# yaito3014/UECRayTracing

Measured on AMD Instinct MI355X. Metric: Msamples/sec at 1920x1080x512spp (~500 spheres); per-pixel RMSE vs CPU, higher is better.
Workload: dtype f64; 1 GPU; BASELINE config 3: 1920x1080x512spp, max_depth 50, RTIOW final scene (485 spheres, generator seed 42), seed0 404, mt19937 + FP64 bit-exact; image=1920x1080, spp=512, max_depth=50, spheres=485

## Files before the change

### uecraytracing_amd/csrc/yk_bvh.cpp

```cpp
#include "yk_bvh.hpp"

#include <algorithm>
#include <cmath>
#include <numeric>

namespace ykbvh {
namespace {

struct Box {
  double lo[3] = {INFINITY, INFINITY, INFINITY};
  double hi[3] = {-INFINITY, -INFINITY, -INFINITY};
  void grow(const Box& b) {
    for (int k = 0; k < 3; ++k) {
      lo[k] = std::min(lo[k], b.lo[k]);
      hi[k] = std::max(hi[k], b.hi[k]);
    }
  }
  void grow(const double* p) {
    for (int k = 0; k < 3; ++k) {
      lo[k] = std::min(lo[k], p[k]);
      hi[k] = std::max(hi[k], p[k]);
    }
  }
  double area() const {
    if (!(hi[0] >= lo[0])) return 0;
    const double dx = hi[0] - lo[0], dy = hi[1] - lo[1], dz = hi[2] - lo[2];
    return 2 * (dx * dy + dy * dz + dz * dx);
  }
};

struct Builder {
  const double* c;
  std::vector<Box> sbox;
  std::vector<double> cent;
  std::vector<uint32_t> idx;
  std::vector<Node> nodes;
  bool median_only = false;
  uint32_t max_depth = 0;
  Options opt;

  Box bounds(uint32_t b, uint32_t e) const {
    Box r;
    for (uint32_t i = b; i < e; ++i) r.grow(sbox[idx[i]]);
    return r;
  }

  int32_t rec(uint32_t b, uint32_t e, uint32_t depth) {
    const uint32_t n = e - b;
    if (n <= opt.max_leaf) {
      max_depth = std::max(max_depth, depth);
      return ~int32_t((b << 4) | n);
    }
    Box cb;
    for (uint32_t i = b; i < e; ++i) cb.grow(&cent[3 * idx[i]]);
    int axis = 0;
    for (int k = 1; k < 3; ++k)
      if (cb.hi[k] - cb.lo[k] > cb.hi[axis] - cb.lo[axis]) axis = k;
    uint32_t mid = b + n / 2;
    double ext = cb.hi[axis] - cb.lo[axis];
    if (!median_only && ext > 0) {
      const int kBins = std::min(std::max(opt.bins, 2), 256);
      double best = INFINITY;
      int best_q = -1, best_axis = axis;
      for (int ax = 0; ax < 3; ++ax) {
        if (!opt.all_axes && ax != axis) continue;
        const double ex = cb.hi[ax] - cb.lo[ax];
        if (!(ex > 0)) continue;
        std::vector<Box> bb(kBins);
        std::vector<uint32_t> cnt(kBins, 0);
        for (uint32_t i = b; i < e; ++i) {
          const uint32_t sp = idx[i];
          const int q = std::min(std::max(int((cent[3 * sp + ax] - cb.lo[ax]) / ex * kBins), 0), kBins - 1);
          bb[q].grow(sbox[sp]);
          ++cnt[q];
        }
        for (int q = 1; q < kBins; ++q) {
          Box l, r;
          uint32_t nl = 0, nr = 0;
          for (int t = 0; t < q; ++t) { l.grow(bb[t]); nl += cnt[t]; }
          for (int t = q; t < kBins; ++t) { r.grow(bb[t]); nr += cnt[t]; }
          if (!nl || !nr) continue;
          const double cost = l.area() * nl + r.area() * nr;
          if (cost < best) { best = cost; best_q = q; best_axis = ax; }
        }
      }
      axis = best_axis;
      ext = cb.hi[axis] - cb.lo[axis];
      auto bin_of = [&](uint32_t sp) {
        int q = int((cent[3 * sp + axis] - cb.lo[axis]) / ext * kBins);
        return std::min(std::max(q, 0), kBins - 1);
      };
      if (best_q > 0) {
        auto it = std::partition(idx.begin() + b, idx.begin() + e,
                                 [&](uint32_t sp) { return bin_of(sp) < best_q; });
        mid = uint32_t(it - idx.begin());
      }
    }
    if (mid == b || mid == e || median_only || ext == 0) {
      mid = b + n / 2;
      std::nth_element(idx.begin() + b, idx.begin() + mid, idx.begin() + e,
                       [&](uint32_t x, uint32_t y) { return cent[3 * x + axis] < cent[3 * y + axis]; });
    }
    const int32_t me = int32_t(nodes.size());
    nodes.emplace_back();
    const int32_t l = rec(b, mid, depth + 1);
    const int32_t r = rec(mid, e, depth + 1);
    const Box bl = bounds(b, mid), br = bounds(mid, e);
    Node& nd = nodes[me];
    const Box* kids[2] = {&bl, &br};
    for (int k = 0; k < 2; ++k) {
      auto dn = [](double v) { float f = (float)v; return (double)f > v ? std::nextafter(f, -INFINITY) : f; };
      auto up = [](double v) { float f = (float)v; return (double)f < v ? std::nextafter(f, INFINITY) : f; };
      nd.lo_x[k] = dn(kids[k]->lo[0]);
      nd.lo_y[k] = dn(kids[k]->lo[1]);
      nd.lo_z[k] = dn(kids[k]->lo[2]);
      nd.hi_x[k] = up(kids[k]->hi[0]);
      nd.hi_y[k] = up(kids[k]->hi[1]);
      nd.hi_z[k] = up(kids[k]->hi[2]);
    }
    nd.child[0] = l;
    nd.child[1] = r;
    nd.pad[0] = nd.pad[1] = 0;
    return me;
  }
};

}

Built build(const double* centers, const double* radii, uint32_t n, double camera_extent,
            const Options& opt) {
  Built out;
  double ext = camera_extent;
  for (uint32_t i = 0; i < n; ++i)
    for (int k = 0; k < 3; ++k) ext = std::max(ext, std::fabs(centers[3 * i + k]) + std::fabs(radii[i]));
  out.origin_bound = 4.0 * ext;
  out.delta = (float)std::ldexp(out.origin_bound, -21);
  for (int attempt = 0; attempt < 2; ++attempt) {
    Builder bd;
    bd.c = centers;
    bd.median_only = attempt == 1;
    bd.opt = opt;
    bd.sbox.resize(n);
    bd.cent.assign(centers, centers + 3 * size_t(n));
    bd.idx.resize(n);
    std::iota(bd.idx.begin(), bd.idx.end(), 0u);
    for (uint32_t i = 0; i < n; ++i) {
      const double ar = std::fabs(radii[i]);
      double g = ar * opt.radius_grow;
      if (opt.f32_big) {
        const double* c = centers + 3 * i;
        const double reach = std::sqrt(3.0) * out.origin_bound + std::sqrt(c[0] * c[0] + c[1] * c[1] + c[2] * c[2]) + ar;
        if (kF32BigReach * ar >= reach * (1.0 + 0x1p-20)) g = std::min(g, ar * kF32BigGrow);
      }
      const double r = ar + g + out.delta;
      for (int k = 0; k < 3; ++k) {
        bd.sbox[i].lo[k] = centers[3 * i + k] - r;
        bd.sbox[i].hi[k] = centers[3 * i + k] + r;
      }
    }
    out.root = bd.rec(0, n, 0);
    out.depth = bd.max_depth;
    if (out.depth <= kMaxDepth || attempt == 1) {
      out.nodes = std::move(bd.nodes);
      out.order = std::move(bd.idx);
      break;
    }
  }
  return out;
}


namespace {
struct Slot {
  float lo[3], hi[3];
  int32_t code;
};

float slot_area(const Slot& e) {
  const float dx = e.hi[0] - e.lo[0], dy = e.hi[1] - e.lo[1], dz = e.hi[2] - e.lo[2];
  return dx * dy + dy * dz + dz * dx;
}

Slot child_slot(const Node& n, int k) {
  return Slot{{n.lo_x[k], n.lo_y[k], n.lo_z[k]}, {n.hi_x[k], n.hi_y[k], n.hi_z[k]}, n.child[k]};
}

double box_area(const float* lo, const float* hi) {
  const double dx = (double)hi[0] - lo[0], dy = (double)hi[1] - lo[1], dz = (double)hi[2] - lo[2];
  return dx * dy + dy * dz + dz * dx;
}

double box_dist2(const float* lo, const float* hi, const double* p) {
  double d2 = 0;
  for (int a = 0; a < 3; ++a) {
    const double d = p[a] < lo[a] ? lo[a] - p[a] : (p[a] > hi[a] ? p[a] - hi[a] : 0.0);
    d2 += d * d;
  }
  return d2;
}

bool box_spans(const float* lo, const float* hi, const float* node_lo, const float* node_hi) {
  return box_area(lo, hi) >= kSpanArea * box_area(node_lo, node_hi);
}

struct Collapser {
  const Built& b;
  const WideOptions& opt;
  std::vector<WideNode>& out;
  std::vector<uint32_t> leaves;
  uint32_t max_depth = 0;

  uint32_t count_leaves(int32_t code) {
    if (code < 0) return 1;
    if (leaves.empty()) leaves.assign(b.nodes.size(), 0);
    if (leaves[code]) return leaves[code];
    return leaves[code] = count_leaves(b.nodes[code].child[0]) + count_leaves(b.nodes[code].child[1]);
  }
  double score(const Slot& e) {
    const double a = slot_area(e);
    if (opt.expand == 0) return a;
    const double nl = count_leaves(e.code);
    return opt.expand == 1 ? a * nl : a * std::sqrt(nl);
  }

  void order_slots(std::vector<Slot>& slots) const {
    if (!opt.view || opt.order == SlotOrder::kTree) return;
    float nlo[3] = {3e38f, 3e38f, 3e38f}, nhi[3] = {-3e38f, -3e38f, -3e38f};
    for (const Slot& e : slots)
      for (int a = 0; a < 3; ++a) {
        nlo[a] = std::min(nlo[a], e.lo[a]);
        nhi[a] = std::max(nhi[a], e.hi[a]);
      }
    struct Key {
      int low;
      double d2;
      Slot slot;
    };
    auto before = [](const Key& x, const Key& y) { return x.low != y.low ? x.low > y.low : x.d2 > y.d2; };
    Key keys[4];
    size_t n = 0;
    for (const Slot& e : slots) {
      const bool leaf = e.code < 0;
      const bool low = opt.order == SlotOrder::kNearLeavesLow
                           ? leaf
                           : (opt.order == SlotOrder::kNearSpanLow && leaf && box_spans(e.lo, e.hi, nlo, nhi));
      const Key key{low ? 1 : 0, box_dist2(e.lo, e.hi, opt.view), e};
      size_t at = n++;
      for (; at > 0 && before(key, keys[at - 1]); --at) keys[at] = keys[at - 1];
      keys[at] = key;
    }
    for (size_t k = 0; k < n; ++k) slots[k] = keys[k].slot;
  }

  uint32_t collapse(int32_t idx, uint32_t depth) {
    std::vector<Slot> slots = {child_slot(b.nodes[idx], 0), child_slot(b.nodes[idx], 1)};
    while (slots.size() < 4) {
      int best = -1;
      for (size_t i = 0; i < slots.size(); ++i)
        if (slots[i].code >= 0 && (best < 0 || score(slots[i]) > score(slots[best]))) best = (int)i;
      if (best < 0) break;
      const Node& c = b.nodes[slots[best].code];
      slots[best] = child_slot(c, 0);
      slots.insert(slots.begin() + best + 1, child_slot(c, 1));
    }
    order_slots(slots);
    max_depth = std::max(max_depth, depth + 1);
    const uint32_t me = (uint32_t)out.size();
    out.emplace_back();
    int32_t codes[4];
    for (int k = 0; k < 4; ++k) {
      if (k >= (int)slots.size()) {
        codes[k] = kEmptyLeaf;
      } else if (slots[k].code >= 0) {
        codes[k] = (int32_t)(collapse(slots[k].code, depth + 1) * sizeof(WideNode));
      } else {
        codes[k] = slots[k].code;
      }
    }
    WideNode& w = out[me];
    float* ax[3] = {w.x, w.y, w.z};
    for (int k = 0; k < 4; ++k) {
      const bool used = k < (int)slots.size();
      for (int a = 0; a < 3; ++a) {
        const float lo = used ? slots[k].lo[a] : 3e38f, hi = used ? slots[k].hi[a] : -3e38f;
        ax[a][k] = lo;
        ax[a][4 + k] = hi;
        ax[a][8 + k] = lo;
      }
      w.child[k] = codes[k];
    }
    return me;
  }
};

void slot_box(const WideNode& w, int k, float* lo, float* hi) {
  const float* ax[3] = {w.x, w.y, w.z};
  for (int a = 0; a < 3; ++a) {
    lo[a] = ax[a][k];
    hi[a] = ax[a][4 + k];
  }
}
}

bool slot_spans(const WideNode& w, int k) {
  float nlo[3] = {3e38f, 3e38f, 3e38f}, nhi[3] = {-3e38f, -3e38f, -3e38f}, lo[3], hi[3];
  for (int j = 0; j < 4; ++j) {
    slot_box(w, j, lo, hi);
    if (!(lo[0] <= hi[0])) continue;
    for (int a = 0; a < 3; ++a) {
      nlo[a] = std::min(nlo[a], lo[a]);
      nhi[a] = std::max(nhi[a], hi[a]);
    }
  }
  slot_box(w, k, lo, hi);
  return lo[0] <= hi[0] && box_spans(lo, hi, nlo, nhi);
}

double slot_dist2(const WideNode& w, int k, const double* p) {
  float lo[3], hi[3];
  slot_box(w, k, lo, hi);
  return box_dist2(lo, hi, p);
}

std::vector<WideNode> wide_nodes(const Built& b, int32_t* root_code, uint32_t* wide_depth,
                                 const WideOptions& wopt) {
  std::vector<WideNode> out;
  uint32_t depth = 0;
  if (b.root >= 0) {
    Collapser c{b, wopt, out, {}, 0};
    c.collapse(b.root, 0);
    depth = c.max_depth;
    *root_code = 0;
  } else {
    *root_code = b.root;
  }
  *wide_depth = depth;
  return out;
}

}
```

### uecraytracing_amd/csrc/yk_context.hip

```cpp
#include <hip/hip_runtime.h>

#include <algorithm>
#include <chrono>
#include <cmath>
#include <cstdio>
#include <cstdlib>
#include <cstring>
#include <string>
#include <vector>

#include "../../include/ykgpu.h"
#include "yk_host_internal.hpp"
#include "yk_schedule.hpp"

using namespace ykhost;

namespace {

thread_local std::string g_last_error;

__global__ void yk_mat_prep(SphereMat* m, uint32_t n) {
  const uint32_t i = blockIdx.x * blockDim.x + threadIdx.x;
  if (i < n) {
    m[i].inv_r = ykd::rcp_refined(m[i].radius);
    m[i].inv_rf = ykf::rcp_refined((float)m[i].radius);
  }
}

}

namespace ykhost {

int fail(int code, const std::string& msg) {
  g_last_error = msg;
  return code;
}
std::string& last_error() { return g_last_error; }

uint64_t device_bytes(const ykgpu_context* ctx) {
  uint64_t b = ctx->t64.bytes + ctx->t32.bytes;
  if (ctx->d_geo) b += (uint64_t)ctx->nspheres * (sizeof(SphereGeo) + sizeof(SphereMat) + sizeof(float4));
  b += ctx->warm_cap + ctx->col_cap * sizeof(double) + ctx->acc_cap * sizeof(double);
  b += ctx->retry_cap * sizeof(uint4);
  b += (uint64_t)ctx->order_slots * sizeof(uint32_t) + (uint64_t)ctx->counter_cap * sizeof(uint32_t);
  b += kCounters * sizeof(unsigned long long);
  if (ctx->d_mt) b += 2ull * ctx->scratch_lanes * ykd::kMtN * sizeof(uint32_t);
  if (ctx->d_ids) b += 2ull * ctx->id_lanes * ctx->id_stride * sizeof(uint16_t);
  b += ctx->rgb_cap + ctx->sums_cap * sizeof(double);
  b += (uint64_t)ctx->cast_cap * (sizeof(yk_ray) + sizeof(yk_hit));
  if (ctx->d_cast_counters) b += (uint64_t)kCastStripes * kCastCounters * sizeof(unsigned long long);
  b += (uint64_t)ctx->rad_cap * (sizeof(yk_path_ray) + sizeof(yk_radiance));
  if (ctx->d_rad_x397) b += kRadChunk * sizeof(uint32_t) + sizeof(uint32_t);
  b += (uint64_t)ctx->rad_mt_lanes * ykd::kMtN * sizeof(uint32_t);
  b += (uint64_t)ctx->rad_lanes * ctx->rad_id_stride * sizeof(uint16_t);
  if (ctx->d_rad_counters) b += (uint64_t)kRadStripes * kRadCounters * sizeof(unsigned long long);
  return b;
}

int finish_stats(ykgpu_context* ctx) {
  if (!ctx->stats_pending) return YK_OK;
  YK_HIP(hipEventSynchronize(ctx->ev1));
  float ms = 0;
  YK_HIP(hipEventElapsedTime(&ms, ctx->ev0, ctx->ev1));
  unsigned long long c[kCounters];
  YK_HIP(hipMemcpy(c, ctx->d_stats, sizeof(c), hipMemcpyDeviceToHost));
  ctx->stats.node_visits = c[4];
  ctx->stats.linear_scans = c[5];
  ctx->stats.newton_calls = c[6];
  ctx->stats.newton_iters = c[7];
  for (int k = 0; k < 8; ++k) ctx->stats.phase_cycles[k] = c[8 + k];
  for (int k = 0; k < 3; ++k) ctx->stats.timeline[k] = c[16 + k];
  for (int k = 0; k < 4; ++k) ctx->stats.diag[k] = c[19 + k];
  for (int k = 0; k < 8; ++k) ctx->stats.work[k] = c[24 + k];
  ctx->stats.total_ms = ms;
  double tw = 0, tr = 0, tp = 0, busy = 0;
  for (uint32_t k = 0; k + 5 < ctx->lev_used; k += 6) {
    float a = 0, b = 0, c = 0;
    YK_HIP(hipEventSynchronize(ctx->lev[k + 5]));
    YK_HIP(hipEventElapsedTime(&a, ctx->lev[k], ctx->lev[k + 1]));
    YK_HIP(hipEventElapsedTime(&b, ctx->lev[k + 2], ctx->lev[k + 3]));
    YK_HIP(hipEventElapsedTime(&c, ctx->lev[k + 4], ctx->lev[k + 5]));
    tw += a, tr += b, tp += c;
    float ov = 0;
    if (k >= 6) YK_HIP(hipEventElapsedTime(&ov, ctx->lev[k + 2], ctx->lev[k - 6 + 3]));
    busy += b - std::min<double>(b, std::max<double>(0.0, ov));
  }
  ctx->stats.render_busy_ms = busy;
  const uint32_t nl = ctx->lev_used / 6;
  std::vector<unsigned long long> clk(4ull * nl);
  std::vector<double> mhz(nl, 0.0);
  if (nl) YK_HIP(hipMemcpy(clk.data(), ctx->d_clk, clk.size() * sizeof(unsigned long long), hipMemcpyDeviceToHost));
  double cyc = 0, real = 0;
  for (uint32_t k = 0; k < nl; ++k) {
    const double dc = (double)(clk[4 * k + 2] - clk[4 * k]), dr = (double)(clk[4 * k + 3] - clk[4 * k + 1]);
    if (dr > 0 && clk[4 * k + 3] > clk[4 * k + 1]) {
      mhz[k] = dc / dr * 100.0;
      cyc += dc;
      real += dr;
    }
  }
  ctx->stats.sclk_mhz = real > 0 ? cyc / real * 100.0 : 0.0;
  if (std::getenv("YKGPU_TIMELINE")) {
    for (uint32_t k = 0; k + 5 < ctx->lev_prev_used && k + 5 < ctx->lev_prev.size(); k += 6) {
      float t[6];
      bool ok = true;
      for (int q = 0; q < 6 && ok; ++q) ok = hipEventElapsedTime(&t[q], ctx->ev0, ctx->lev_prev[k + q]) == hipSuccess;
      if (!ok) {
        (void)hipGetLastError();
        break;
      }
      std::fprintf(stderr, "prev   %u: warm %8.3f %8.3f  render %8.3f %8.3f  reduce %8.3f %8.3f\n", k / 6, t[0],
                   t[1], t[2], t[3], t[4], t[5]);
    }
    for (uint32_t k = 0; k + 5 < ctx->lev_used; k += 6) {
      float t[6];
      for (int q = 0; q < 6; ++q) YK_HIP(hipEventElapsedTime(&t[q], ctx->ev0, ctx->lev[k + q]));
      std::fprintf(stderr, "launch %u: warm %8.3f %8.3f  render %8.3f %8.3f  reduce %8.3f %8.3f  sclk %7.1f MHz\n",
                   k / 6, t[0], t[1], t[2], t[3], t[4], t[5], mhz[k / 6]);
    }
    std::fprintf(stderr, "call %8.3f\n", ms);
  }
  ctx->stats.warmup_ms = tw;
  ctx->stats.kernel_ms = tr;
  ctx->stats.resolve_ms = tp;
  ctx->stats.segments = c[0];
  ctx->stats.sphere_tests = c[1];
  ctx->stats.sqrt_calls = c[2];
  ctx->stats.mt_fallbacks = c[3];
  ctx->stats.device_bytes = device_bytes(ctx);
  ctx->stats_pending = false;
  return YK_OK;
}

}

namespace {

int upload_tree(ykgpu_context* ctx, DevTree& t, const std::vector<double>& centers, const std::vector<double>& radii,
                double cam_ext, const ykbvh::Options& opt, uint32_t leaf_cap, const void* geo, size_t elem,
                size_t tgeo_elem, const RenderKernel (&kern)[2][2], bool exact_stack,
                const ykbvh::WideOptions& wopt) {
  const uint32_t count = (uint32_t)radii.size();
  if (opt.max_leaf > leaf_cap) return fail(YK_ERR_UNSUPPORTED, "BVH leaf size above the kernel's leaf capacity");
  const ykbvh::Built bvh = ykbvh::build(centers.data(), radii.data(), count, cam_ext, opt);
  if (bvh.depth > ykbvh::kMaxDepth) return fail(YK_ERR_INVALID, "BVH deeper than the traversal stack");
  std::vector<char> leaf_geo(count * elem);
  for (uint32_t i = 0; i < count; ++i)
    std::memcpy(leaf_geo.data() + i * elem, (const char*)geo + (size_t)bvh.order[i] * elem, elem);
  t.release();
  int32_t root_code = 0;
  uint32_t wdepth = 0;
  const std::vector<DevNode> snodes = ykbvh::wide_nodes(bvh, &root_code, &wdepth, wopt);
  auto leaf_fits = [&](int32_t code) { return code >= 0 || (((~(uint32_t)code) & 15u) <= leaf_cap); };
  bool fits = leaf_fits(root_code);
  for (const DevNode& w : snodes)
    for (int k = 0; k < 4; ++k) fits = fits && leaf_fits(w.child[k]);
  if (!fits) return fail(YK_ERR_UNSUPPORTED, "a BVH leaf holds more spheres than the kernel's leaf code tests");
  const size_t nn = std::max<size_t>(1, snodes.size());
  YK_HIP(hipMalloc(&t.nodes, nn * sizeof(DevNode)));
  YK_HIP(hipMalloc(&t.leaf_geo, count * elem));
  YK_HIP(hipMalloc(&t.leaf_ids, count * sizeof(uint32_t)));
  if (!snodes.empty())
    YK_HIP(hipMemcpy(t.nodes, snodes.data(), snodes.size() * sizeof(DevNode), hipMemcpyHostToDevice));
  YK_HIP(hipMemcpy(t.leaf_geo, leaf_geo.data(), count * elem, hipMemcpyHostToDevice));
  YK_HIP(hipMemcpy(t.leaf_ids, bvh.order.data(), count * sizeof(uint32_t), hipMemcpyHostToDevice));
  t.bytes = nn * sizeof(DevNode) + count * elem + count * sizeof(uint32_t);
  t.root = root_code;
  t.depth = bvh.depth;
  t.wide_depth = wdepth;
  t.origin_bound = bvh.origin_bound;
  t.n_nodes = (uint32_t)snodes.size();
  auto a16 = [](size_t b) { return (b + 15) & ~size_t(15); };
  const size_t scene_bytes = a16(t.n_nodes * sizeof(DevNode)) + a16(count * elem) + a16(count * sizeof(uint32_t));
  const size_t tgeo_bytes = tgeo_elem ? a16(count * tgeo_elem) : 0;
  const size_t mat_bytes = tgeo_elem ? a16(count * sizeof(SphereMat)) : 0;
  t.geo_off = (uint32_t)a16(t.n_nodes * sizeof(DevNode));
  t.ids_off = t.geo_off + (uint32_t)a16(count * elem);
  for (int v = 0; v < 2; ++v) {
    DevTree::Plan& pl = t.plan[v];
    const int blk = block_of(v == 1);
    const int rays = blk;
    const size_t budget = (size_t)160 * 1024 / (blk >= 512 ? 1 : 768 / blk) - 2048;
    const size_t min_stacks = (size_t)12 * rays * 4;
    pl.in_lds = scene_bytes + tgeo_bytes + mat_bytes + min_stacks <= budget;
    const size_t tables = pl.in_lds ? tgeo_bytes + mat_bytes : 0;
    {
      const size_t used = pl.in_lds ? scene_bytes + tables : 0;
      const uint32_t fit = used + min_stacks <= budget ? (uint32_t)((budget - used) / (rays * 4)) : 12u;
      pl.stack_cap = std::max(8u, std::min(3 * wdepth + 1, fit - 4));
      pl.stack_entries = pl.stack_cap + 4;
      pl.stack_check = true;
      if (exact_stack && fit >= 3 * wdepth + 1) {
        pl.stack_cap = 3 * wdepth + 1;
        pl.stack_entries = pl.stack_cap;
        pl.stack_check = false;
      }
#ifdef YK_STACK_CAP_FORCE
      pl.stack_cap = YK_STACK_CAP_FORCE;
      pl.stack_entries = pl.stack_cap + 4;
      pl.stack_check = true;
#endif
    }
    pl.tgeo_off = pl.in_lds && tgeo_elem ? (uint32_t)scene_bytes : 0u;
    pl.mat_off = pl.in_lds && tgeo_elem ? (uint32_t)(scene_bytes + tgeo_bytes) : 0u;
    pl.stack_off = pl.in_lds ? (uint32_t)(scene_bytes + tables) : 0u;
    pl.lds_bytes = pl.stack_off + pl.stack_entries * rays * (uint32_t)sizeof(int32_t);
    int per_cu = 0;
    const RenderKernel k = kern[v][pl.in_lds ? 1 : 0];
    const hipError_t e = hipOccupancyMaxActiveBlocksPerMultiprocessor(&per_cu, k, blk, pl.lds_bytes);
    if (e != hipSuccess || per_cu < 1) per_cu = 1;
    pl.grid = per_cu * ctx->cus;
  }
  return YK_OK;
}

}

extern "C" {

uint32_t ykgpu_abi_version(void) { return YKGPU_ABI_VERSION; }

const char* ykgpu_last_error(void) { return g_last_error.c_str(); }

int ykgpu_device_count(int* count) {
  if (!count) return fail(YK_ERR_INVALID, "null count");
  int n = 0;
  hipError_t e = hipGetDeviceCount(&n);
  if (e != hipSuccess) {
    *count = 0;
    return fail(YK_ERR_DEVICE, std::string("hipGetDeviceCount: ") + hipGetErrorString(e));
  }
  *count = n;
  return YK_OK;
}

int ykgpu_context_create(int device, ykgpu_context** out) {
  if (!out) return fail(YK_ERR_INVALID, "null out");
  *out = nullptr;
  int n = 0;
  if (hipGetDeviceCount(&n) != hipSuccess || n == 0)
    return fail(YK_ERR_DEVICE, "no HIP device (the renderer has no CPU fallback)");
  if (device < 0 || device >= n) return fail(YK_ERR_INVALID, "device index out of range");
  YK_HIP(hipSetDevice(device));
  hipDeviceProp_t prop;
  YK_HIP(hipGetDeviceProperties(&prop, device));
  if (std::strncmp(prop.gcnArchName, "gfx950", 6) != 0)
    return fail(YK_ERR_DEVICE, std::string("built for gfx950, device is ") + prop.gcnArchName);
  auto* ctx = new ykgpu_context();
  ctx->device = device;
  ctx->cus = prop.multiProcessorCount;
  for (int k16 = 0; k16 < 16; ++k16)
    (void)hipFuncSetAttribute((const void*)fp64_kernel(k16 & 8, k16 & 7), hipFuncAttributeMaxDynamicSharedMemorySize,
                              160 * 1024);
  for (int k8 = 0; k8 < 8; ++k8)
    (void)hipFuncSetAttribute((const void*)f32_kernel(k8 & 4, (k8 & 1) | ((k8 & 2) << 1)),
                              hipFuncAttributeMaxDynamicSharedMemorySize, 160 * 1024);
  if (hipStreamCreateWithFlags(&ctx->stream, hipStreamNonBlocking) != hipSuccess ||
      hipStreamCreateWithFlags(&ctx->aux, hipStreamNonBlocking) != hipSuccess ||
      hipStreamCreateWithFlags(&ctx->red, hipStreamNonBlocking) != hipSuccess ||
      create_render_stream(&ctx->alt) != hipSuccess || create_render_stream(&ctx->ren) != hipSuccess ||
      hipEventCreate(&ctx->ev0) != hipSuccess || hipEventCreate(&ctx->ev1) != hipSuccess ||
      hipMalloc(&ctx->d_stats, kCounters * sizeof(unsigned long long)) != hipSuccess) {
    ykgpu_context_destroy(ctx);
    return fail(YK_ERR_DEVICE, "context resources");
  }
  *out = ctx;
  return YK_OK;
}

int ykgpu_context_destroy(ykgpu_context* ctx) {
  if (!ctx) return YK_OK;
  (void)hipSetDevice(ctx->device);
  if (ctx->stream) (void)hipStreamSynchronize(ctx->stream);
  (void)hipFree(ctx->d_geo);
  (void)hipFree(ctx->d_mat);
  (void)hipFree(ctx->d_geo_f);
  (void)hipFree(ctx->d_counter);
  (void)hipFree(ctx->d_clk);
  (void)hipFree(ctx->d_stats);
  (void)hipFree(ctx->d_warm);
  (void)hipFree(ctx->d_retry);
  (void)hipFree(ctx->d_order);
  (void)hipFree(ctx->d_col);
  (void)hipFree(ctx->d_acc);
  ctx->t64.release();
  ctx->t32.release();
  (void)hipFree(ctx->d_mt);
  (void)hipFree(ctx->d_ids);
  (void)hipFree(ctx->d_rgb);
  (void)hipFree(ctx->d_sums);
  (void)hipFree(ctx->d_cast_rays);
  (void)hipFree(ctx->d_cast_hits);
  (void)hipFree(ctx->d_cast_counters);
  if (ctx->cast_ev) (void)hipEventDestroy(ctx->cast_ev);
  for (void* q : {ctx->d_rad_rays, ctx->d_rad_out, (void*)ctx->d_rad_x397, (void*)ctx->d_rad_claim, (void*)ctx->d_rad_mt,
                  (void*)ctx->d_rad_ids, (void*)ctx->d_rad_counters})
    (void)hipFree(q);
  if (ctx->rad_ev) (void)hipEventDestroy(ctx->rad_ev);
  for (hipEvent_t e : ctx->lev) (void)hipEventDestroy(e);
  for (hipEvent_t e : ctx->lev_prev) (void)hipEventDestroy(e);
  for (hipEvent_t e : ctx->gev) (void)hipEventDestroy(e);
  if (ctx->ev0) (void)hipEventDestroy(ctx->ev0);
  if (ctx->ev1) (void)hipEventDestroy(ctx->ev1);
  if (ctx->stream) (void)hipStreamDestroy(ctx->stream);
  if (ctx->aux) (void)hipStreamDestroy(ctx->aux);
  if (ctx->red) (void)hipStreamDestroy(ctx->red);
  if (ctx->alt) (void)hipStreamDestroy(ctx->alt);
  if (ctx->ren) (void)hipStreamDestroy(ctx->ren);
  delete ctx;
  return YK_OK;
}

int ykgpu_set_scene(ykgpu_context* ctx, const yk_sphere* spheres, uint32_t count,
                    const yk_camera* camera) {
  if (!ctx || !spheres || !camera) return fail(YK_ERR_INVALID, "null argument");
  if (count == 0 || count > 65535) return fail(YK_ERR_INVALID, "sphere count must be 1..65535");
  std::vector<SphereGeo> geo(count);
  std::vector<SphereMat> mat(count);
  std::vector<float4> geo_f(count);
  for (uint32_t i = 0; i < count; ++i) {
    const yk_sphere& s = spheres[i];
    if (s.material > YK_MATERIAL_DIELECTRIC) return fail(YK_ERR_INVALID, "unknown material kind");
    geo[i] = {s.center[0], s.center[1], s.center[2], s.radius * s.radius};
    const float rf = (float)s.radius;
    geo_f[i] = make_float4((float)s.center[0], (float)s.center[1], (float)s.center[2], rf * rf);
    mat[i] = {s.albedo[0], s.albedo[1], s.albedo[2], s.fuzz, s.radius, s.ior, s.material, 0.0f, 0.0};
    if (s.material == YK_MATERIAL_DIELECTRIC) {
      const double inv = 1.0 / s.ior;
      double r0f = (1 - inv) / (1 + inv), r0b = (1 - s.ior) / (1 + s.ior);
      r0f = r0f * r0f;
      r0b = r0b * r0b;
      mat[i].fuzz = inv;
      mat[i].ar = r0f;
      mat[i].ag = r0b;
    }
  }
  YK_HIP(hipSetDevice(ctx->device));
  YK_HIP(hipEventSynchronize(ctx->ev1));
  YK_HIP(hipStreamSynchronize(ctx->stream));
  for (hipStream_t s : {ctx->aux, ctx->red, ctx->ren, ctx->alt}) YK_HIP(hipStreamSynchronize(s));
  if (ctx->cast_ev) YK_HIP(hipEventSynchronize(ctx->cast_ev));
  if (ctx->rad_ev) YK_HIP(hipEventSynchronize(ctx->rad_ev));
  ++ctx->scene_gen;
  if (count > ctx->nspheres || !ctx->d_geo) {
    (void)hipFree(ctx->d_geo);
    (void)hipFree(ctx->d_mat);
    (void)hipFree(ctx->d_geo_f);
    ctx->d_geo = nullptr;
    ctx->d_mat = nullptr;
    ctx->d_geo_f = nullptr;
    YK_HIP(hipMalloc(&ctx->d_geo, count * sizeof(SphereGeo)));
    YK_HIP(hipMalloc(&ctx->d_mat, count * sizeof(SphereMat)));
    YK_HIP(hipMalloc(&ctx->d_geo_f, count * sizeof(float4)));
  }
  YK_HIP(hipMemcpy(ctx->d_geo, geo.data(), count * sizeof(SphereGeo), hipMemcpyHostToDevice));
  YK_HIP(hipMemcpy(ctx->d_geo_f, geo_f.data(), count * sizeof(float4), hipMemcpyHostToDevice));
  std::vector<double> centers(3 * size_t(count)), radii(count);
  double rmin = INFINITY;
  for (uint32_t i = 0; i < count; ++i) {
    for (int k = 0; k < 3; ++k) centers[3 * i + k] = spheres[i].center[k];
    radii[i] = spheres[i].radius;
    rmin = std::min(rmin, std::fabs(radii[i]));
  }
  double cam_ext = 0;
  for (int k = 0; k < 3; ++k) cam_ext = std::max(cam_ext, std::fabs(camera->origin[k]));
  ykbvh::Options bopt;
  bopt.max_leaf = kLeafCapF64;
  if (const char* e = ab_knob("YKGPU_BVH_BINS")) bopt.bins = std::max(2, std::min(256, std::atoi(e)));
  bopt.all_axes = true;
  if (const char* e = ab_knob("YKGPU_BVH_ALLAXES")) bopt.all_axes = std::atoi(e) != 0;
  const RenderKernel k64[2][2] = {{fp64_kernel(false, 0), fp64_kernel(true, 0)},
                                  {fp64_kernel(false, 4), fp64_kernel(true, 4)}};
  ykbvh::WideOptions wopt;
  wopt.view = camera->origin;
  if (const char* e = ab_knob("YKGPU_BVH_ORDER"))
    wopt.order = (ykbvh::SlotOrder)std::max(0, std::min(3, std::atoi(e)));
  int rc = upload_tree(ctx, ctx->t64, centers, radii, cam_ext, bopt, kLeafCapF64, geo.data(), sizeof(SphereGeo),
                       sizeof(SphereGeo), k64, true, wopt);
  if (rc) return rc;
  {
    double dmax = 1.0;
    for (int k = 0; k < 3; ++k)
      dmax = std::max(dmax, std::fabs(camera->lower_left_corner[k]) + std::fabs(camera->horizontal[k]) +
                                std::fabs(camera->vertical[k]) + std::fabs(camera->origin[k]) +
                                std::fabs(camera->lens_radius) *
                                    (std::fabs(camera->lens_u[k]) + std::fabs(camera->lens_v[k])));
    if (!(ctx->t64.origin_bound <= 0x1p27) || !(ctx->t64.origin_bound >= 0x1p-60 * dmax))
      ctx->t64.origin_bound = -1.0;
  }
  ykbvh::Options fopt = bopt;
  fopt.max_leaf = kLeafCapF32;
  if (const char* e = ab_knob("YKGPU_BVH_ALLAXES_F32")) fopt.all_axes = std::atoi(e) != 0;
  fopt.radius_grow = 2.0 * (double)ykbvh::kF32Cone;
  fopt.f32_big = ab_knob("YKGPU_F32_NO_BIG") == nullptr;
  const RenderKernel k32[2][2] = {{f32_kernel(false, 0), f32_kernel(true, 0)},
                                  {f32_kernel(false, 4), f32_kernel(true, 4)}};
  ykbvh::WideOptions fwopt = wopt;
  if (const char* e = ab_knob("YKGPU_BVH_ORDER_F32"))
    fwopt.order = (ykbvh::SlotOrder)std::max(0, std::min(3, std::atoi(e)));
  rc = upload_tree(ctx, ctx->t32, centers, radii, cam_ext, fopt, kLeafCapF32, geo_f.data(), sizeof(float4),
                   sizeof(float4), k32, false, fwopt);
  if (rc) return rc;
  if (!(rmin >= 0x1p-20) || !(ctx->t32.origin_bound <= 0x1p20)) ctx->t32.origin_bound = -1.0;
  YK_HIP(hipMemcpy(ctx->d_mat, mat.data(), count * sizeof(SphereMat), hipMemcpyHostToDevice));
  hipLaunchKernelGGL(yk_mat_prep, dim3((count + 255) / 256), dim3(256), 0, ctx->stream, ctx->d_mat, count);
  YK_HIP(hipGetLastError());
  YK_HIP(hipStreamSynchronize(ctx->stream));
  ctx->nspheres = count;
  ctx->cam = *camera;
  double ext = 0;
  for (uint32_t i = 0; i < count; ++i) {
    const yk_sphere& s = spheres[i];
    const double e = std::fmax(std::fabs(s.center[0]), std::fmax(std::fabs(s.center[1]), std::fabs(s.center[2]))) +
                     std::fabs(s.radius);
    ext = e > ext || e != e ? e : ext;
    if (ext != ext) break;
  }
  ctx->cast_extent = ext;
  ctx->have_scene = true;
  return YK_OK;
}

int ykgpu_render_async(ykgpu_context* ctx, const yk_render_params* p, void* rgb_device,
                       void* stream) {
  int rc = check_params(ctx, p);
  if (rc) return rc;
  if (!rgb_device) return fail(YK_ERR_INVALID, "null output");
  YK_HIP(hipSetDevice(ctx->device));
  hipStream_t st = stream ? (hipStream_t)stream : ctx->stream;
  ctx->t0 = std::chrono::steady_clock::now();
  return launch(ctx, p, (uint8_t*)rgb_device, nullptr, st, 0, p->samples_per_pixel, nullptr);
}

static int render_host(ykgpu_context* ctx, const yk_render_params* p, uint8_t* rgb_host,
                       double* sums_host) {
  int rc = check_params(ctx, p);
  if (rc) return rc;
  YK_HIP(hipSetDevice(ctx->device));
  const auto t0 = std::chrono::steady_clock::now();
  const size_t npix = (size_t)p->row_count * tile_width(p);
  if (npix * 3 > ctx->rgb_cap) {
    (void)hipFree(ctx->d_rgb);
    ctx->d_rgb = nullptr;
    YK_HIP(hipMalloc(&ctx->d_rgb, npix * 3));
    ctx->rgb_cap = npix * 3;
  }
  if (sums_host && npix * 3 > ctx->sums_cap) {
    (void)hipFree(ctx->d_sums);
    ctx->d_sums = nullptr;
    YK_HIP(hipMalloc(&ctx->d_sums, npix * 3 * sizeof(double)));
    ctx->sums_cap = npix * 3;
  }
  rc = launch(ctx, p, ctx->d_rgb, sums_host ? ctx->d_sums : nullptr, ctx->stream, 0, p->samples_per_pixel, nullptr);
  if (rc) return rc;
  if (rgb_host) YK_HIP(hipMemcpyAsync(rgb_host, ctx->d_rgb, npix * 3, hipMemcpyDeviceToHost, ctx->stream));
  if (sums_host)
    YK_HIP(hipMemcpyAsync(sums_host, ctx->d_sums, npix * 3 * sizeof(double), hipMemcpyDeviceToHost,
                          ctx->stream));
  YK_HIP(hipStreamSynchronize(ctx->stream));
  rc = finish_stats(ctx);
  ctx->stats.total_ms =
      std::chrono::duration<double, std::milli>(std::chrono::steady_clock::now() - t0).count();
  return rc;
}

int ykgpu_render(ykgpu_context* ctx, const yk_render_params* p, uint8_t* rgb_host) {
  if (!rgb_host) return fail(YK_ERR_INVALID, "null output");
  return render_host(ctx, p, rgb_host, nullptr);
}

int ykgpu_render_trace(ykgpu_context* ctx, const yk_render_params* p, uint32_t max_rays, double* rays_host,
                       uint32_t* counts_host) {
  int rc = check_params(ctx, p);
  if (rc) return rc;
  if (!max_rays || !rays_host || !counts_host) return fail(YK_ERR_INVALID, "null output or max_rays == 0");
  const size_t n = (size_t)p->row_count * tile_width(p) * p->samples_per_pixel;
  YK_HIP(hipSetDevice(ctx->device));
  YK_HIP(hipMalloc(&ctx->d_trace, n * max_rays * 6 * sizeof(double)));
  if (hipMalloc(&ctx->d_trace_counts, n * sizeof(uint32_t)) != hipSuccess) {
    (void)hipFree(ctx->d_trace);
    ctx->d_trace = nullptr;
    return fail(YK_ERR_NOMEM, "ykgpu_render_trace: ray counts");
  }
  ctx->trace_cap = max_rays;
  yk_render_params q = *p;
  q.flags |= YK_FLAG_COUNT_WORK | YK_FLAG_TRACE_RAYS;
  rc = render_host(ctx, &q, nullptr, nullptr);
  hipError_t e = hipSuccess;
  if (!rc) e = hipMemcpy(rays_host, ctx->d_trace, n * max_rays * 6 * sizeof(double), hipMemcpyDeviceToHost);
  if (!rc && e == hipSuccess) e = hipMemcpy(counts_host, ctx->d_trace_counts, n * sizeof(uint32_t), hipMemcpyDeviceToHost);
  (void)hipFree(ctx->d_trace);
  (void)hipFree(ctx->d_trace_counts);
  ctx->d_trace = nullptr;
  ctx->d_trace_counts = nullptr;
  ctx->trace_cap = 0;
  if (rc) return rc;
  if (e != hipSuccess) return fail(YK_ERR_DEVICE, std::string("ykgpu_render_trace: ") + hipGetErrorString(e));
  return YK_OK;
}

int ykgpu_render_sums(ykgpu_context* ctx, const yk_render_params* p, double* sums_host) {
  if (!sums_host) return fail(YK_ERR_INVALID, "null output");
  return render_host(ctx, p, nullptr, sums_host);
}

int ykgpu_get_stats(ykgpu_context* ctx, yk_render_stats* out) {
  if (!ctx || !out) return fail(YK_ERR_INVALID, "null argument");
  YK_HIP(hipSetDevice(ctx->device));
  int rc = finish_stats(ctx);
  if (rc) return rc;
  *out = ctx->stats;
  return YK_OK;
}

}
```

### uecraytracing_amd/csrc/yk_device.hpp

```cpp
#pragma once

#include <hip/hip_runtime.h>
#include <stdint.h>

namespace ykd {

struct v3 {
  double x, y, z;
};
__device__ __forceinline__ v3 add(v3 a, v3 b) { return {a.x + b.x, a.y + b.y, a.z + b.z}; }
__device__ __forceinline__ v3 sub(v3 a, v3 b) { return {a.x - b.x, a.y - b.y, a.z - b.z}; }
__device__ __forceinline__ v3 mul(v3 a, double s) { return {a.x * s, a.y * s, a.z * s}; }
__device__ __forceinline__ v3 divs(v3 a, double s) { return {a.x / s, a.y / s, a.z / s}; }
__device__ __forceinline__ v3 neg(v3 a) { return {-a.x, -a.y, -a.z}; }
__device__ __forceinline__ double dot(v3 a, v3 b) { return a.x * b.x + a.y * b.y + a.z * b.z; }
__device__ __forceinline__ double len2(v3 a) { return a.x * a.x + a.y * a.y + a.z * a.z; }

__device__ __forceinline__ bool div_range(double x) { return fabs(x) >= 0x1p-400 && fabs(x) <= 0x1p400; }
__device__ __forceinline__ bool num_range(double x) { return x == 0.0 || div_range(x); }
__device__ __forceinline__ double rcp_refined(double s) {
  const double r0 = __builtin_amdgcn_rcp(s);
  double t = __builtin_fma(-s, r0, 1.0);
  const double r1 = __builtin_fma(r0, t, r0);
  t = __builtin_fma(-s, r1, 1.0);
  return __builtin_fma(r1, t, r1);
}
__device__ __forceinline__ double div_by(double n, double s, double r) {
  const double q0 = n * r;
  const double e = __builtin_fma(-s, q0, n);
  return __builtin_copysign(__builtin_fma(e, r, q0), q0);
}
__device__ __forceinline__ double div_pos(double n, double s, double r) {
  const double q0 = n * r;
  return __builtin_fma(__builtin_fma(-s, q0, n), r, q0);
}
__device__ __forceinline__ v3 divs_fast(v3 a, double s) {
  const double r = rcp_refined(s);
  v3 q = {div_by(a.x, s, r), div_by(a.y, s, r), div_by(a.z, s, r)};
  const bool ok = div_range(s) && num_range(a.x) && num_range(a.y) && num_range(a.z);
  if (__builtin_expect(__ballot(!ok) != 0, 0)) q = divs(a, s);
  return q;
}
__device__ __forceinline__ v3 divs_fast_r(v3 a, double s, double r) {
  v3 q = {div_by(a.x, s, r), div_by(a.y, s, r), div_by(a.z, s, r)};
  const bool ok = div_range(s) && num_range(a.x) && num_range(a.y) && num_range(a.z);
  if (__builtin_expect(__ballot(!ok) != 0, 0)) q = divs(a, s);
  return q;
}
__device__ __forceinline__ double div_markstein(double n, double d, double y) {
  const double q0 = n * y;
  return __builtin_fma(__builtin_fma(-d, q0, n), y, q0);
}

__device__ __forceinline__ double sqrt_bound(double x) {
  const double r = __builtin_amdgcn_rsq(x);
  const double y = x * r, h = 0.5 * r;
  const double y1 = __builtin_fma(__builtin_fma(-y, y, x), h, y);
  return x == 0.0 ? 0.0 : y1;
}
__device__ __forceinline__ double rcp_bound(double a) {
  const double r0 = __builtin_amdgcn_rcp(a);
  return __builtin_fma(r0, __builtin_fma(-a, r0, 1.0), r0);
}
__device__ __forceinline__ double sqrt_start(double s) {
  const double r = __builtin_amdgcn_rsq(s);
  double g = s * r, h = r * 0.5;
  const double e = __builtin_fma(-h, g, 0.5);
  g = __builtin_fma(g, e, g);
  h = __builtin_fma(h, e, h);
  double d = __builtin_fma(-g, g, s);
  g = __builtin_fma(d, h, g);
  d = __builtin_fma(-g, g, s);
  return __builtin_fma(d, h, g);
}

__device__ __forceinline__ double nsqrt_impl(double s, uint32_t& iters) {
  double x, prev = 0.0;
  if (s >= 0x1p-400 && s <= 0x1p400) {
    x = sqrt_start(s);
    ++iters;
    return (x + div_pos(s, x, rcp_refined(x))) / 2.0;
  }
  x = (s >= 0x1p-1000 && s <= 0x1.fffffffffffffp+1023) ? __builtin_sqrt(s) : s / 2.0;
  for (int guard = 0; x != prev && guard < 4096; ++guard) {
    prev = x;
    x = (x + s / x) / 2.0;
    ++iters;
  }
  return x;
}
__device__ __forceinline__ double nsqrt(double s) {
  uint32_t it = 0;
  return nsqrt_impl(s, it);
}

__device__ __forceinline__ double nsqrt_c(double s, uint32_t& calls, uint32_t& iters) {
  ++calls;
  return nsqrt_impl(s, iters);
}

__device__ __forceinline__ v3 normalized(v3 a) { return divs(a, nsqrt(len2(a))); }
__device__ __forceinline__ v3 reflect(v3 v, v3 n) { return sub(v, mul(n, 2.0 * dot(v, n))); }
__device__ __forceinline__ bool near_zero(v3 a) {
  const double ax = a.x > 0 ? a.x : -a.x, ay = a.y > 0 ? a.y : -a.y;
  return (ax < 1e-8) && (ay < 1e-8) && (ax < 1e-8);
}

constexpr uint32_t kMtN = 624, kMtM = 397, kLazyDraws = kMtN - kMtM;

__device__ __forceinline__ uint32_t mt_seed_step(uint32_t prev, uint32_t i) {
  return 1812433253u * (prev ^ (prev >> 30)) + i;
}
__device__ __forceinline__ uint32_t xor_and(uint32_t a, uint32_t b, uint32_t c) {
  return __builtin_amdgcn_bitop3_b32(a, b, c, 0x78);
}
__device__ __forceinline__ uint32_t mt_mix(uint32_t hi_src, uint32_t lo_src) {
  const uint32_t y = __builtin_amdgcn_bitop3_b32(hi_src, lo_src, 0x80000000u, 0xE4);
  const uint32_t odd = 0u - (lo_src & 1u);
  return xor_and(y >> 1, odd, 0x9908b0dfu);
}
__device__ __forceinline__ uint32_t mt_temper(uint32_t z) {
  z ^= (z >> 11);
  z = xor_and(z, z << 7, 0x9d2c5680u);
  z = xor_and(z, z << 15, 0xefc60000u);
  z ^= (z >> 18);
  return z;
}

struct MtLane {
  uint32_t a0, a1, b;
  uint32_t j;
  uint32_t seed;
  uint32_t* state;
};
__device__ __forceinline__ bool mt_used_fallback(const MtLane& g) { return g.j > kLazyDraws; }
__device__ __forceinline__ uint32_t rng_words(const MtLane& g) { return g.j; }
__device__ __forceinline__ uint32_t rng_twists(const MtLane& g) { return g.j > kLazyDraws ? 1u + (g.j - 1u) / kMtN : 0u; }

__device__ __forceinline__ void mt_start(MtLane& g, uint32_t seed) {
  g.seed = seed;
  g.j = 0;
  g.a0 = seed;
  uint32_t x = mt_seed_step(seed, 1);
  g.a1 = x;
#pragma unroll 8
  for (uint32_t i = 2; i <= kMtM; ++i) x = mt_seed_step(x, i);
  g.b = x;
}

__device__ __forceinline__ void mt_start_from(MtLane& g, uint32_t seed, uint32_t x397) {
  g.seed = seed;
  g.j = 0;
  g.a0 = seed;
  g.a1 = mt_seed_step(seed, 1);
  g.b = x397;
}

#ifndef YK_WALK_MAD
#define YK_WALK_MAD 1
#endif
__device__ __forceinline__ uint32_t mt_seed_step_mad(uint32_t prev, uint64_t i, uint32_t cmul) {
  const uint32_t t = prev ^ (prev >> 30);
  uint64_t r, carry;
  asm("v_mad_u64_u32 %0, %1, %2, %3, %4" : "=v"(r), "=s"(carry) : "v"(t), "v"(cmul), "s"(i));
  return (uint32_t)r;
}

template <int N>
__device__ __forceinline__ void mt_walk397xn(uint32_t (&x)[N]) {
#pragma unroll
  for (int k = 0; k < N; ++k) x[k] = mt_seed_step(x[k], 1);
#if YK_WALK_MAD
  uint32_t cmul;
  asm("v_mov_b32 %0, 0x6c078965" : "=v"(cmul));
#pragma unroll 4
  for (uint32_t i = 2; i <= kMtM; ++i) {
#pragma unroll
    for (int k = 0; k < N; ++k) x[k] = mt_seed_step_mad(x[k], (uint64_t)i, cmul);
  }
#else
#pragma unroll 4
  for (uint32_t i = 2; i <= kMtM; ++i) {
#pragma unroll
    for (int k = 0; k < N; ++k) x[k] = mt_seed_step(x[k], i);
  }
#endif
}

constexpr uint32_t kMtSeedMulInv = 0x9638806du;
__device__ __forceinline__ uint32_t mt_seed_from(uint32_t x, uint32_t i) {
  for (; i > 0; --i) {
    const uint32_t t = (x - i) * kMtSeedMulInv;
    x = t ^ (t >> 30);
  }
  return x;
}
__device__ __noinline__ uint32_t mt_slow(uint32_t* st, uint32_t x227, uint32_t j) {
  const uint32_t idx = j % kMtN;
  if (j == kLazyDraws) {
    uint32_t x = mt_seed_from(x227, kLazyDraws);
    st[0] = x;
    for (uint32_t i = 1; i < kMtN; ++i) {
      x = mt_seed_step(x, i);
      st[i] = x;
    }
  }
  if (j == kLazyDraws || idx == 0) {
    uint32_t k = 0;
    for (; k < kMtN - kMtM; ++k) st[k] = st[k + kMtM] ^ mt_mix(st[k], st[k + 1]);
    for (; k < kMtN - 1; ++k) st[k] = st[k + kMtM - kMtN] ^ mt_mix(st[k], st[k + 1]);
    st[kMtN - 1] = st[kMtM - 1] ^ mt_mix(st[kMtN - 1], st[0]);
  }
  return st[idx];
}

__device__ __forceinline__ uint32_t mt_next_lazy(MtLane& g) {
  const uint32_t z = g.b ^ mt_mix(g.a0, g.a1);
  g.a0 = g.a1;
  g.a1 = mt_seed_step(g.a1, g.j + 2);
  g.b = mt_seed_step(g.b, g.j + kMtM + 1);
  ++g.j;
  return mt_temper(z);
}
__device__ __forceinline__ bool rng_lazy_ok(const MtLane& g, uint32_t words) { return g.j + words <= kLazyDraws; }

__device__ __forceinline__ uint32_t mt_next(MtLane& g) {
  uint32_t z;
  if (g.j < kLazyDraws) {
    z = g.b ^ mt_mix(g.a0, g.a1);
    g.a0 = g.a1;
    g.a1 = mt_seed_step(g.a1, g.j + 2);
    g.b = mt_seed_step(g.b, g.j + kMtM + 1);
  } else {
    z = mt_slow(g.state, g.a0, g.j);
  }
  ++g.j;
  return mt_temper(z);
}

__device__ __forceinline__ uint32_t sample_seed(uint32_t mode, uint64_t key, uint32_t seed0, uint32_t y,
                                                uint32_t x, uint32_t W, uint32_t spp, uint32_t s) {
#ifndef YK_SEED_COUNTER_ONLY
  if (mode == 1u) {
    uint64_t z = key + (((uint64_t)y * W + x) * spp + s + 1) * 0x9E3779B97F4A7C15ull;
    z = (z ^ (z >> 30)) * 0xBF58476D1CE4E5B9ull;
    z = (z ^ (z >> 27)) * 0x94D049BB133111EBull;
    z ^= z >> 31;
    return (uint32_t)(z >> 32);
  }
#endif
  return seed0 + (y * W + x) * spp + s;
}

struct X128Lane {
  uint32_t x, y, z, w;
  uint32_t n;
};
__device__ __forceinline__ void x128_start(X128Lane& g, uint32_t seed) {
  g.x = 123456789u;
  g.y = 362436069u;
  g.z = 521288629u;
  g.w = 88675123u ^ seed;
  g.n = 0;
}
__device__ __forceinline__ uint32_t x128_next(X128Lane& g) {
  const uint32_t t = g.x ^ (g.x << 11);
  g.x = g.y;
  g.y = g.z;
  g.z = g.w;
  g.w = (g.w ^ (g.w >> 19)) ^ (t ^ (t >> 8));
  ++g.n;
  return g.w;
}
__device__ __forceinline__ bool mt_used_fallback(const X128Lane&) { return false; }
__device__ __forceinline__ uint32_t rng_words(const X128Lane& g) { return g.n; }
__device__ __forceinline__ uint32_t rng_twists(const X128Lane&) { return 0u; }

__device__ __forceinline__ bool rng_lazy_ok(const X128Lane&, uint32_t) { return true; }

template <bool kLazy = false>
__device__ __forceinline__ uint32_t rng_next(MtLane& g) { return kLazy ? mt_next_lazy(g) : mt_next(g); }
template <bool kLazy = false>
__device__ __forceinline__ uint32_t rng_next(X128Lane& g) { return x128_next(g); }

template <bool kLazy = false, class G>
__device__ __forceinline__ double canonical(G& g) {
  const double u0 = (double)rng_next<kLazy>(g);
  const double u1 = (double)rng_next<kLazy>(g);
  double r = __builtin_fma(u1, 0x1p-32, u0 * 0x1p-64);
  if (r >= 1.0) r = 1.0 - 0x1p-53;
  return r;
}
template <bool kLazy = false, class G>
__device__ __forceinline__ double uniform(G& g, double a, double b) {
  return (canonical<kLazy>(g) * (b - a)) + a;
}
__device__ __forceinline__ double uniform_of(double c, double a, double b) {
  if (a == -1.0 && b == 1.0) return __builtin_fma(c, 2.0, -1.0);
  if (a == 0.0 && b == 1.0) return c;
  return (c * (b - a)) + a;
}
__device__ __forceinline__ bool rng_can_speculate(const MtLane& g) { return g.j + 2 <= kLazyDraws; }
__device__ __forceinline__ bool rng_can_speculate(const X128Lane&) { return true; }
template <class G>
__device__ __forceinline__ v3 random_vec(G& g, double lo, double hi) {
  v3 r;
  r.x = uniform(g, lo, hi);
  r.y = uniform(g, lo, hi);
  r.z = uniform(g, lo, hi);
  return r;
}

__device__ __forceinline__ double reflectance_r0(double cosine, double r0) {
  const double x = 1 - cosine;
  return r0 + (1 - r0) * ((((x * x) * x) * x) * x);
}

}
```

### uecraytracing_amd/csrc/yk_host_internal.hpp

```cpp
#ifndef YK_HOST_INTERNAL_HPP
#define YK_HOST_INTERNAL_HPP

#include <hip/hip_runtime.h>

#include <chrono>
#include <cstdint>
#include <map>
#include <string>
#include <vector>

#include "../../include/ykgpu.h"
#include "yk_render_device.hpp"

namespace ykhost {
int fail(int code, const std::string& msg);
std::string& last_error();
}

#define YK_HIP(call)                                                                      \
  do {                                                                                    \
    hipError_t e_ = (call);                                                               \
    if (e_ != hipSuccess)                                                                 \
      return ykhost::fail(e_ == hipErrorOutOfMemory ? YK_ERR_NOMEM : YK_ERR_DEVICE,       \
                          std::string(#call) + ": " + hipGetErrorString(e_));             \
  } while (0)

struct DevTree {
  DevNode* nodes = nullptr;
  void* leaf_geo = nullptr;
  uint32_t* leaf_ids = nullptr;
  int32_t root = 0;
  uint32_t depth = 0, n_nodes = 0;
  uint32_t wide_depth = 0;
  double origin_bound = 0;
  uint32_t geo_off = 0, ids_off = 0;
  size_t bytes = 0;
  struct Plan {
    bool in_lds = false;
    uint32_t lds_bytes = 0, stack_off = 0, stack_cap = 0, stack_entries = 0;
    bool stack_check = true;
    uint32_t tgeo_off = 0, mat_off = 0;
    int grid = 0;
  } plan[2];
  void release() {
    (void)hipFree(nodes);
    (void)hipFree(leaf_geo);
    (void)hipFree(leaf_ids);
    nodes = nullptr;
    leaf_geo = nullptr;
    leaf_ids = nullptr;
    bytes = 0;
  }
};

constexpr int kCastCounters = 8, kCastStripes = 64;
constexpr int kRadCounters = 8, kRadStripes = 64;
constexpr uint64_t kRadChunk = 1ull << 22;

struct ykgpu_context {
  int device = 0;
  int cus = 0;
  DevTree t64, t32;
  size_t scratch_lanes = 0;
  char* d_warm = nullptr;
  uint4* d_retry = nullptr;
  size_t retry_cap = 0;
  double* d_col = nullptr;
  double* d_acc = nullptr;
  size_t col_cap = 0, acc_cap = 0;
  uint32_t* d_order = nullptr;
  uint32_t order_w = 0, order_rows = 0, order_slots = 0, order_stride = 0, order_mode = 0;
  size_t warm_cap = 0;
  hipStream_t stream = nullptr;
  hipStream_t aux = nullptr;
  hipStream_t red = nullptr;
  hipStream_t alt = nullptr;
  hipStream_t ren = nullptr;
  hipEvent_t ev0 = nullptr, ev1 = nullptr;
  std::vector<hipEvent_t> lev;
  uint32_t lev_used = 0;
  std::vector<hipEvent_t> lev_prev;
  uint32_t lev_prev_used = 0;
  uint32_t prev_n = 0;
  std::vector<hipEvent_t> gev;
  uint64_t run_len = 0;
  struct RingGeom {
    uint64_t nps = 0, K = 0, welem = 0, warm_ring = 0, col_ring = 0, lanes = 0, id_stride = 0;
    const void *warm = nullptr, *col = nullptr, *mt = nullptr, *ids = nullptr;
    bool operator==(const RingGeom& o) const {
      return nps == o.nps && K == o.K && welem == o.welem && warm_ring == o.warm_ring && col_ring == o.col_ring &&
             lanes == o.lanes && id_stride == o.id_stride && warm == o.warm && col == o.col && mt == o.mt &&
             ids == o.ids;
    }
  } prev_geom;
  uint64_t prev_shape = 0;
  bool prev_ok = false;
  bool prev_enqueued = false;
  bool dirty = false;
  uint64_t g_next = 0;
  SphereGeo* d_geo = nullptr;
  SphereMat* d_mat = nullptr;
  float4* d_geo_f = nullptr;
  uint32_t nspheres = 0;
  yk_camera cam{};
  bool have_scene = false;
  uint64_t scene_gen = 0;
  uint32_t* d_counter = nullptr;
  uint32_t counter_cap = 0;
  unsigned long long* d_clk = nullptr;
  unsigned long long* d_stats = nullptr;
  uint32_t* d_mt = nullptr;
  uint16_t* d_ids = nullptr;
  uint32_t id_stride = 0;
  size_t id_lanes = 0;
  uint8_t* d_rgb = nullptr;
  size_t rgb_cap = 0;
  double* d_sums = nullptr;
  size_t sums_cap = 0;
  yk_render_stats stats{};
  bool stats_pending = false;
  double* d_trace = nullptr;
  uint32_t* d_trace_counts = nullptr;
  uint32_t trace_cap = 0;
  std::chrono::steady_clock::time_point t0;
  double cast_extent = 0;
  void* d_cast_rays = nullptr;
  void* d_cast_hits = nullptr;
  size_t cast_cap = 0;
  unsigned long long* d_cast_counters = nullptr;
  hipEvent_t cast_ev = nullptr;
  yk_cast_stats cast_stats{};
  void* d_rad_rays = nullptr;
  void* d_rad_out = nullptr;
  size_t rad_cap = 0;
  uint32_t* d_rad_x397 = nullptr;
  uint32_t* d_rad_claim = nullptr;
  uint32_t* d_rad_mt = nullptr;
  uint16_t* d_rad_ids = nullptr;
  size_t rad_lanes = 0, rad_id_stride = 0, rad_mt_lanes = 0;
  unsigned long long* d_rad_counters = nullptr;
  hipEvent_t rad_ev = nullptr;
  yk_radiance_stats rad_stats{};
};

struct ykgpu_film {
  ykgpu_context* ctx = nullptr;
  int device = 0;
  yk_render_params p{};
  uint64_t scene_gen = 0;
  uint32_t done = 0;
  uint32_t nps = 0;
  uint64_t npix = 0;
  double* d_plane = nullptr;
  uint32_t* d_order = nullptr;
  unsigned long long* d_result = nullptr;
  std::vector<uint32_t> order;
  bool torn = false;
  std::map<uint32_t, uint64_t> hist;
  uint32_t* d_count = nullptr;
  uint32_t* d_take = nullptr;
  uint32_t* d_blocks = nullptr;
  uint32_t* d_gorder = nullptr;
  uint32_t* d_gmap = nullptr;
  unsigned long long* d_hist = nullptr;
  uint32_t g_slots = 0;
  void* d_denoise = nullptr;
  void* d_features = nullptr;
  uint32_t feature_grid = 0;
  bool uniform() const { return hist.size() <= 1; }
};

struct ykgpu_group {
  std::vector<ykgpu_context*> ctx;
  std::vector<uint8_t*> tile;
  std::vector<size_t> tile_cap;
  std::vector<yk_render_stats> st;
  yk_render_stats total{};
};

struct ykgpu_group_film {
  ykgpu_group* g = nullptr;
  yk_render_params p{};
  uint32_t k = 0, wt = 0;
  std::vector<ykgpu_film*> film;
  std::vector<uint32_t> rows;
  std::vector<uint64_t> gen;
  std::vector<ykgpu_film*> band;
  uint32_t halo = 0;
  bool have_bands = false;
  bool torn = false;
};

namespace {
inline RenderKernel fp64_kernel(bool lds, int mode) { return (RenderKernel)yk_fp64_kernel(lds, mode); }
inline RenderKernel f32_kernel(bool lds, int mode) { return (RenderKernel)yk_f32_kernel(lds, mode); }
}

namespace ykhost {

int check_params(const ykgpu_context* ctx, const yk_render_params* p);
uint32_t tile_width(const yk_render_params* p);
uint64_t host_row_y(const yk_render_params* p, uint32_t t);
uint64_t host_col_x(const yk_render_params* p, uint32_t j);
uint32_t order_mode();
uint32_t order_stride(const yk_render_params* p);
std::vector<uint32_t> build_order(uint32_t W, uint32_t rows, uint32_t stride, uint32_t mode);
hipError_t create_render_stream(hipStream_t* s);
int launch(ykgpu_context* ctx, const yk_render_params* p, uint8_t* rgb_dev, double* sums_dev, hipStream_t st,
           uint32_t s_begin, uint32_t s_end, ykgpu_film* film);
uint64_t device_bytes(const ykgpu_context* ctx);
int finish_stats(ykgpu_context* ctx);
int film_ready(const ykgpu_film* film);
int film_accumulate_enqueue(ykgpu_film* film, uint32_t n_samples);
int film_accumulate_finish(ykgpu_film* film, uint32_t n_samples, std::chrono::steady_clock::time_point t0);
int denoise_params_check(const yk_denoise_params& dp);
int feature_params_check(const yk_feature_params& fp);
struct DenoiseBufs {
  double *mv, *out;
  uint8_t* rgb;
  unsigned long long* low;
};
int denoise_buffers(ykgpu_film* film, DenoiseBufs* out);
hipError_t denoise_moments_enqueue(ykgpu_film* film, const DenoiseBufs& b);
hipError_t denoise_band_enqueue(ykgpu_film* band, const DenoiseBufs& b, const yk_denoise_params& dp,
                                const yk_feature_params* fp, const double* feat, uint32_t r0, uint32_t n, bool want_rgb);
int yk_film_features_ensure(ykgpu_film* film, uint32_t grid, const double** planes, double* ms);

inline const uint32_t* film_counts(const ykgpu_film* film) { return film->uniform() ? nullptr : film->d_count; }
inline bool film_consecutive(const ykgpu_film* film) {
  const yk_render_params& p = film->p;
  return host_row_y(&p, p.row_count - 1) == (uint64_t)p.row_begin + p.row_count - 1 &&
         host_col_x(&p, tile_width(&p) - 1) == (uint64_t)p.col_begin + tile_width(&p) - 1;
}
struct TileCols {
  uint32_t begin, stride, band;
};
inline TileCols film_cols(const ykgpu_film* film) {
  const yk_render_params& p = film->p;
  return p.col_count ? TileCols{p.col_begin, p.col_stride, p.col_band_log2} : TileCols{0, 1, 0};
}

}

#endif
```

### uecraytracing_amd/csrc/yk_pipeline.hip

```cpp
#include <hip/hip_runtime.h>

#include <algorithm>
#include <cmath>
#include <cstdlib>
#include <random>
#include <string>
#include <vector>

#include "../../include/ykgpu.h"
#include "yk_film_internal.hpp"
#include "yk_host_internal.hpp"
#include "yk_schedule.hpp"

namespace {

struct WarmArgs {
  uint32_t W, spp, seed0, row_begin, row_stride, s0, npix_slots, seed_mode, band_log2;
  uint32_t Wt, col_begin, col_stride, col_band;
  uint32_t nps_m, nps_sh, w_m, w_sh;
  uint32_t lens, H;
  uint64_t seed_key;
  yk_camera cam;
  CamF camf;
  double w_d, h_d, inv_w, inv_h;
  const uint32_t* order;
  uint64_t n;
  void* out;
  uint32_t* counter;
  uint4* retry;
  uint32_t retry_cap, retry_pad;
};

inline uint32_t retry_cap_for(uint64_t slots_per_wave) {
  const double m = 0.2146 * (double)slots_per_wave, sd = std::sqrt(m * 0.7854);
  return ((uint32_t)(m + 6.0 * sd) + 64u + 63u) & ~63u;
}
__device__ __forceinline__ void retry_put(uint4* r, uint32_t i, const ykd::MtLane& g, double uc, double vc) {
  r[0] = make_uint4(i, g.seed, g.a0, g.a1);
  r[1] = make_uint4(g.b, g.j, 0u, 0u);
  *(double2*)(r + 2) = make_double2(uc, vc);
}
__device__ __forceinline__ uint64_t ld_l2(const uint4* r, int k) {
  return __hip_atomic_load((const uint64_t*)r + k, __ATOMIC_RELAXED, __HIP_MEMORY_SCOPE_AGENT);
}
__device__ __forceinline__ uint32_t retry_get(const uint4* r, ykd::MtLane& g, double& uc, double& vc) {
  const uint64_t w0 = ld_l2(r, 0), w1 = ld_l2(r, 1), w2 = ld_l2(r, 2);
  g.state = nullptr;
  g.seed = (uint32_t)(w0 >> 32);
  g.a0 = (uint32_t)w1;
  g.a1 = (uint32_t)(w1 >> 32);
  g.b = (uint32_t)w2;
  g.j = (uint32_t)(w2 >> 32);
  uc = __longlong_as_double((long long)ld_l2(r, 4));
  vc = __longlong_as_double((long long)ld_l2(r, 5));
  return (uint32_t)w0;
}

template <bool kLens, bool kF32, bool kDefer, uint32_t kIlp>
__device__ __forceinline__ void mt_warmup_body(const WarmArgs& wa) {
  constexpr uint32_t kWarmBlock = 256;
  const uint32_t n = (uint32_t)wa.n;
  const uint32_t stride = gridDim.x * kWarmBlock;
  if (blockIdx.x == 0 && threadIdx.x == 0) *wa.counter = 0u;
  static_assert(!kDefer || (kLens && !kF32), "the deferred lens loop is the FP64 lens warm-up's");
  uint4* const ring =
      kDefer ? wa.retry + (size_t)__builtin_amdgcn_readfirstlane((blockIdx.x * kWarmBlock + threadIdx.x) >> 6) *
                              wa.retry_cap * 3
             : nullptr;
  uint32_t rcount = 0;
  auto slot_seed = [&](uint32_t i, uint32_t& xx, uint32_t& y) -> uint32_t {
    const uint32_t sl = fdiv(i, wa.nps_m, wa.nps_sh), pp = i - sl * wa.npix_slots;
    const uint32_t q = wa.order[pp];
    const uint32_t pix = q == kNoPixel ? 0u : q;
    const uint32_t tr = fdiv(pix, wa.w_m, wa.w_sh);
    xx = tile_col_x(wa.col_begin, wa.col_stride, wa.col_band, pix - tr * wa.Wt);
    y = tile_row_y(wa.row_begin, wa.row_stride, wa.band_log2, tr);
    const uint32_t seed = ykd::sample_seed(wa.seed_mode, wa.seed_key, wa.seed0, y, xx, wa.W, wa.spp, wa.s0 + sl);
    xx = q == kNoPixel ? kPadX : xx;
    return seed;
  };
  auto start_slot = [&](uint32_t i, uint32_t xx, uint32_t y, uint32_t seed, uint32_t x397) {
    ykd::MtLane g;
    g.state = nullptr;
    ykd::mt_start_from(g, seed, x397);
    bool failed = false;
    if constexpr (kF32) {
      const float uc = ykf::canonical<true>(g);
      const float vc = ykf::canonical<true>(g);
      float px = 0.0f, py = 0.0f;
      if (kLens) {
        for (;;) {
          if (!ykd::rng_lazy_ok(g, 2)) {
            failed = true;
            break;
          }
          px = ykf::uniform_of(ykf::canonical<true>(g), -1.0f, 1.0f);
          py = ykf::uniform_of(ykf::canonical<true>(g), -1.0f, 1.0f);
          if (px * px + py * py < 1.0f) break;
        }
      }
      ykf::v3 o, d;
      camera_ray_f32(wa.camf, wa.H, xx, y, uc, vc, kLens, px, py, o, d);
      uint4* const out = (uint4*)wa.out + 3 * (size_t)i;
      *(float4*)out = make_float4(o.x, o.y, o.z, d.x);
      *(float4*)(out + 1) = make_float4(d.y, d.z, 0.0f, 0.0f);
      out[2] = make_uint4(g.a0, g.a1, g.b, xx == kPadX ? kPadSlot : failed ? kNoStart : g.j);
    } else {
      const double uc = ykd::canonical<true>(g);
      const double vc = ykd::canonical<true>(g);
      double px = 0.0, py = 0.0;
      if constexpr (kDefer) {
        bool again = false;
        if (!ykd::rng_lazy_ok(g, 4)) {
          failed = true;
        } else {
          px = ykd::uniform<true>(g, -1, 1);
          py = ykd::uniform<true>(g, -1, 1);
          again = !(px * px + py * py < 1.0);
        }
        const unsigned long long m = __ballot(again);
        const uint32_t nq = (uint32_t)__popcll(m);
        const bool room = rcount + nq <= wa.retry_cap;
        if (room) {
          if (again) {
            const uint32_t pos = rcount + __builtin_amdgcn_mbcnt_hi((uint32_t)(m >> 32), __builtin_amdgcn_mbcnt_lo((uint32_t)m, 0u));
            retry_put(ring + 3 * pos, i, g, uc, vc);
          }
          rcount += nq;
          if (again) return;
        } else if (again) {
          failed = true;
        }
      } else if (kLens) {
        for (;;) {
          if (!ykd::rng_lazy_ok(g, 4)) {
            failed = true;
            break;
          }
          px = ykd::uniform<true>(g, -1, 1);
          py = ykd::uniform<true>(g, -1, 1);
          if (px * px + py * py < 1.0) break;
        }
      }
      v3 o, d;
      camera_ray(wa.cam, wa.w_d, wa.inv_w, wa.h_d, wa.inv_h, wa.H, xx, y, uc, vc, kLens, px, py, o, d);
      uint4* const out = (uint4*)wa.out + 4 * (size_t)i;
      *(double2*)out = make_double2(o.x, o.y);
      *(double2*)(out + 1) = make_double2(o.z, d.x);
      *(double2*)(out + 2) = make_double2(d.y, d.z);
      out[3] = make_uint4(g.a0, g.a1, g.b, xx == kPadX ? kPadSlot : failed ? kNoStart : g.j);
    }
  };
  if constexpr (kIlp > 1) {
    for (uint32_t i = blockIdx.x * kWarmBlock + threadIdx.x; i < n; i += kIlp * stride) {
      uint32_t xx, y, x[kIlp];
#pragma unroll
      for (uint32_t k = kIlp - 1; k > 0; --k) {
        const uint32_t ik = i + k * stride;
        x[k] = slot_seed(ik < n ? ik : i, xx, y);
      }
      const uint32_t seed = slot_seed(i, xx, y);
      x[0] = seed;
      ykd::mt_walk397xn<kIlp>(x);
      start_slot(i, xx, y, seed, x[0]);
#pragma unroll
      for (uint32_t k = 1; k < kIlp; ++k) {
        const uint32_t ik = i + k * stride;
        if (ik < n) {
          const uint32_t sk = slot_seed(ik, xx, y);
          start_slot(ik, xx, y, sk, x[k]);
        }
      }
    }
  } else {
    for (uint32_t i = blockIdx.x * kWarmBlock + threadIdx.x; i < n; i += stride) {
      uint32_t xx, y;
      const uint32_t seed = slot_seed(i, xx, y);
      uint32_t x[1] = {seed};
      ykd::mt_walk397xn<1>(x);
      start_slot(i, xx, y, seed, x[0]);
    }
  }
  if constexpr (kDefer) {
    const uint32_t lane = threadIdx.x & 63u;
    uint32_t head = 0, cnt = __builtin_amdgcn_readfirstlane(rcount);
    asm volatile("s_waitcnt vmcnt(0)" ::: "memory");
    while (cnt > 0u) {
      const uint32_t take = min(cnt, 64u);
      const bool act = lane < take;
      ykd::MtLane g;
      double uc = 0, vc = 0, px = 0, py = 0;
      uint32_t i = 0;
      bool again = false, failed = false;
      if (act) {
        uint32_t pos = head + lane;
        pos = pos >= wa.retry_cap ? pos - wa.retry_cap : pos;
        i = retry_get(ring + 3 * pos, g, uc, vc);
        if (!ykd::rng_lazy_ok(g, 4)) {
          failed = true;
        } else {
          px = ykd::uniform<true>(g, -1, 1);
          py = ykd::uniform<true>(g, -1, 1);
          again = !(px * px + py * py < 1.0);
        }
      }
      head += take;
      head = head >= wa.retry_cap ? head - wa.retry_cap : head;
      cnt -= take;
      const unsigned long long m = __ballot(again);
      if (again) {
        uint32_t pos = head + cnt + __builtin_amdgcn_mbcnt_hi((uint32_t)(m >> 32), __builtin_amdgcn_mbcnt_lo((uint32_t)m, 0u));
        pos = pos >= wa.retry_cap ? pos - wa.retry_cap : pos;
        retry_put(ring + 3 * pos, i, g, uc, vc);
      }
      cnt += (uint32_t)__popcll(m);
      if (act && !again) {
        const uint32_t sl = fdiv(i, wa.nps_m, wa.nps_sh), pp = i - sl * wa.npix_slots;
        const uint32_t q = wa.order[pp];
        const uint32_t pix = q == kNoPixel ? 0u : q;
        const uint32_t tr = fdiv(pix, wa.w_m, wa.w_sh);
        const uint32_t xx = tile_col_x(wa.col_begin, wa.col_stride, wa.col_band, pix - tr * wa.Wt);
        const uint32_t y = tile_row_y(wa.row_begin, wa.row_stride, wa.band_log2, tr);
        uint4* const out = (uint4*)wa.out + 4 * (size_t)i;
        out[3] = make_uint4(g.a0, g.a1, g.b, q == kNoPixel ? kPadSlot : failed ? kNoStart : g.j);
        v3 o, d;
        camera_ray(wa.cam, wa.w_d, wa.inv_w, wa.h_d, wa.inv_h, wa.H, xx, y, uc, vc, kLens, px, py, o, d);
        *(double2*)out = make_double2(o.x, o.y);
        *(double2*)(out + 1) = make_double2(o.z, d.x);
        *(double2*)(out + 2) = make_double2(d.y, d.z);
      }
      if (cnt > 0u) asm volatile("s_waitcnt vmcnt(0)" ::: "memory");
    }
  }
}

template <bool kLens, bool kF32>
__global__ __launch_bounds__(256) void yk_mt_warmup(WarmArgs wa) {
  mt_warmup_body<kLens, kF32, false, 1>(wa);
}
__global__ __launch_bounds__(256) __attribute__((amdgpu_num_vgpr(YK_DEFER_VGPRS / 2))) void yk_mt_warmup_defer(WarmArgs wa) {
  mt_warmup_body<true, false, true, kWalkIlp>(wa);
}

struct ReduceArgs {
  const double* col;
  double* acc;
  const uint32_t* order;
  uint8_t* rgb;
  double* sums;
  uint32_t npix_slots, nsl, ks, spp;
  uint32_t first, last, pad0, pad1;
};
__device__ __forceinline__ void reduce_slot(const ReduceArgs& ra, uint32_t p) {
  const uint32_t q = ra.order[p];
  if (q == kNoPixel) return;
  double a[3];
#pragma unroll
  for (int c = 0; c < 3; ++c) a[c] = ra.first ? 0.0 : ra.acc[(size_t)c * ra.npix_slots + p];
  for (uint32_t k = 0; k < ra.ks; ++k) {
    const size_t i = (size_t)k * ra.npix_slots + p;
#pragma unroll
    for (int c = 0; c < 3; ++c) a[c] = a[c] + ra.col[i * kColStride + c];
  }
  if (!ra.last) {
#pragma unroll
    for (int c = 0; c < 3; ++c) ra.acc[(size_t)c * ra.npix_slots + p] = a[c];
    return;
  }
  const size_t o3 = (size_t)q * 3;
  const double spp = (double)ra.spp;
#pragma unroll
  for (int c = 0; c < 3; ++c) {
    if (ra.sums) ra.sums[o3 + c] = a[c];
    double v = ykd::nsqrt(a[c] / spp);
    v = (v < 0.0) ? 0.0 : (0.999 < v) ? 0.999 : v;
    ra.rgb[o3 + c] = (uint8_t)(uint32_t)(v * 256);
  }
}
__global__ __launch_bounds__(256) void yk_reduce_samples(ReduceArgs ra) {
  for (uint32_t p = blockIdx.x * blockDim.x + threadIdx.x; p < ra.npix_slots; p += gridDim.x * blockDim.x)
    reduce_slot(ra, p);
}

struct FilmReduceArgs {
  const double* col;
  double* plane;
  const uint32_t* order;
  uint32_t npix_slots, ks;
};
__global__ __launch_bounds__(256) void yk_film_reduce(FilmReduceArgs fa) {
  for (uint32_t p = blockIdx.x * blockDim.x + threadIdx.x; p < fa.npix_slots; p += gridDim.x * blockDim.x) {
    if (fa.order[p] == kNoPixel) continue;
    double s[3], q[3];
#pragma unroll
    for (int c = 0; c < 3; ++c) {
      s[c] = fa.plane[(size_t)c * fa.npix_slots + p];
      q[c] = fa.plane[(size_t)(3 + c) * fa.npix_slots + p];
    }
    for (uint32_t k = 0; k < fa.ks; ++k) {
      const double* rec = fa.col + ((size_t)k * fa.npix_slots + p) * kColStride;
#pragma unroll
      for (int c = 0; c < 3; ++c) {
        const double v = rec[c];
        s[c] = film_add(s[c], v);
        q[c] = film_add(q[c], film_mul(v, v));
      }
    }
#pragma unroll
    for (int c = 0; c < 3; ++c) {
      fa.plane[(size_t)c * fa.npix_slots + p] = s[c];
      fa.plane[(size_t)(3 + c) * fa.npix_slots + p] = q[c];
    }
  }
}

struct FilmMaskedArgs {
  const double* col;
  double* plane;
  uint32_t* count;
  uint32_t* take;
  const uint32_t* map;
  uint32_t npix_slots, g_slots, ks, pad;
};
__global__ __launch_bounds__(256) void yk_film_reduce_masked(FilmMaskedArgs fa) {
  for (uint32_t a = blockIdx.x * blockDim.x + threadIdx.x; a < fa.g_slots; a += gridDim.x * blockDim.x) {
    const uint32_t p = fa.map[a];
    if (p >= fa.npix_slots) continue;
    double s[3], q[3];
#pragma unroll
    for (int c = 0; c < 3; ++c) {
      s[c] = fa.plane[(size_t)c * fa.npix_slots + p];
      q[c] = fa.plane[(size_t)(3 + c) * fa.npix_slots + p];
    }
    for (uint32_t k = 0; k < fa.ks; ++k) {
      const double* rec = fa.col + ((size_t)k * fa.g_slots + a) * kColStride;
#pragma unroll
      for (int c = 0; c < 3; ++c) {
        const double v = rec[c];
        s[c] = film_add(s[c], v);
        q[c] = film_add(q[c], film_mul(v, v));
      }
    }
#pragma unroll
    for (int c = 0; c < 3; ++c) {
      fa.plane[(size_t)c * fa.npix_slots + p] = s[c];
      fa.plane[(size_t)(3 + c) * fa.npix_slots + p] = q[c];
    }
    fa.count[p] += fa.ks;
    if (fa.take) fa.take[p] = 0u;
  }
}

}

static_assert(kLaunchBytes / (8 * kColStride) * 4 < (1ull << 32), "4 * slot must fit 32 bits");
static_assert(yksched::kColourBytes == kColStride * sizeof(double), "yk_schedule.hpp's colour record");

namespace ykhost {

uint64_t host_row_y(const yk_render_params* p, uint32_t t) {
  const uint32_t L = p->row_band_log2;
  return (uint64_t)p->row_begin + ((((uint64_t)(t >> L)) * p->row_stride) << L) + (t & ((1u << L) - 1u));
}

uint32_t tile_width(const yk_render_params* p) { return p->col_count ? p->col_count : p->image_width; }
uint64_t host_col_x(const yk_render_params* p, uint32_t j) {
  if (!p->col_count) return j;
  const uint32_t L = p->col_band_log2;
  return (uint64_t)p->col_begin + ((((uint64_t)(j >> L)) * p->col_stride) << L) + (j & ((1u << L) - 1u));
}

static void fastdiv(uint32_t d, uint32_t& m, uint32_t& sh) {
  uint32_t l = 0;
  while ((1ull << l) < d) ++l;
  sh = 31 + l;
  m = (uint32_t)(((1ull << sh) + d - 1) / d);
}

int check_params(const ykgpu_context* ctx, const yk_render_params* p) {
  if (!ctx || !p) return fail(YK_ERR_INVALID, "null context or params");
  if (!ctx->have_scene) return fail(YK_ERR_NO_SCENE, "ykgpu_set_scene was not called");
  if (!p->image_width || !p->image_height || !p->samples_per_pixel)
    return fail(YK_ERR_INVALID, "image_width, image_height and samples_per_pixel must be > 0");
  if (!p->row_count) return fail(YK_ERR_INVALID, "row_count must be > 0");
  if (!p->row_stride) return fail(YK_ERR_INVALID, "row_stride must be > 0");
  if (p->row_band_log2 > 10) return fail(YK_ERR_INVALID, "row_band_log2 must be <= 10");
  if (host_row_y(p, p->row_count - 1) >= p->image_height) return fail(YK_ERR_INVALID, "row range outside the image");
  if (p->col_count) {
    if (!p->col_stride) return fail(YK_ERR_INVALID, "col_stride must be > 0");
    if (p->col_band_log2 > 10) return fail(YK_ERR_INVALID, "col_band_log2 must be <= 10");
    if (host_col_x(p, p->col_count - 1) >= p->image_width) return fail(YK_ERR_INVALID, "column range outside the image");
  } else if (p->col_begin || p->col_stride || p->col_band_log2) {
    return fail(YK_ERR_INVALID, "col_count == 0 (every column) needs col_begin, col_stride, col_band_log2 == 0");
  }
  if ((uint64_t)p->row_count * tile_width(p) >= (1ull << 31))
    return fail(YK_ERR_INVALID, "tile larger than 2^31 pixels");
  if (p->precision != YK_PRECISION_FP64 && p->precision != YK_PRECISION_FP32)
    return fail(YK_ERR_UNSUPPORTED, "precision mode");
  if (p->rng != YK_RNG_MT19937 && p->rng != YK_RNG_XOR128) return fail(YK_ERR_UNSUPPORTED, "rng mode");
  if (p->seed_mode != YK_SEED_COUNTER && p->seed_mode != YK_SEED_RANDOM_DEVICE)
    return fail(YK_ERR_UNSUPPORTED, "seed mode");
  if (!(p->t_min >= 0)) return fail(YK_ERR_INVALID, "t_min must be >= 0");
  if ((p->flags & YK_FLAG_ONE_LANE) &&
      (!(p->flags & YK_FLAG_COUNT_WORK) || p->precision != YK_PRECISION_FP64))
    return fail(YK_ERR_INVALID, "YK_FLAG_ONE_LANE needs YK_FLAG_COUNT_WORK and FP64");
  return YK_OK;
}

static int quiesce(ykgpu_context* ctx) {
  for (hipStream_t s : {ctx->aux, ctx->red, ctx->ren, ctx->alt, ctx->stream}) YK_HIP(hipStreamSynchronize(s));
  return YK_OK;
}

static int ensure_scratch(ykgpu_context* ctx, uint32_t max_depth, size_t lanes, bool need_mt) {
  if (need_mt && (lanes > ctx->scratch_lanes || !ctx->d_mt)) {
    if (int rc = quiesce(ctx)) return rc;
    (void)hipFree(ctx->d_mt);
    ctx->d_mt = nullptr;
    ctx->scratch_lanes = 0;
    YK_HIP(hipMalloc(&ctx->d_mt, 2 * lanes * ykd::kMtN * sizeof(uint32_t)));
    ctx->scratch_lanes = lanes;
  }
  const uint32_t need = max_depth > kStackRegs ? max_depth : 1;
  if (need > ctx->id_stride || lanes > ctx->id_lanes || !ctx->d_ids) {
    if (int rc = quiesce(ctx)) return rc;
    if (ctx->d_ids) YK_HIP(hipFree(ctx->d_ids));
    ctx->d_ids = nullptr;
    ctx->id_stride = 0;
    ctx->id_lanes = 0;
    YK_HIP(hipMalloc(&ctx->d_ids, 2 * lanes * need * sizeof(uint16_t)));
    ctx->id_stride = need;
    ctx->id_lanes = lanes;
  }
  return YK_OK;
}

uint32_t order_mode() {
  const char* oe = ab_knob("YKGPU_ORDER");
  return oe ? (uint32_t)std::atoi(oe) : 0u;
}
uint32_t order_stride(const yk_render_params* p) {
  return p->row_count > 1 && p->row_band_log2 < 3 ? p->row_stride : 1;
}
std::vector<uint32_t> build_order(uint32_t W, uint32_t rows, uint32_t stride, uint32_t mode) {
  std::vector<uint32_t> ord;
  if (kTile == 0) {
    ord.resize((size_t)W * rows);
    for (size_t i = 0; i < ord.size(); ++i) ord[i] = (uint32_t)i;
  } else {
    const uint32_t th = stride <= 1 ? kTile : (stride <= 4 ? std::max(1u, kTile / 2) : std::max(1u, kTile / 4));
    const uint32_t tw = kTile * kTile / th;
    const uint32_t bx = (W + tw - 1) / tw, by = (rows + th - 1) / th;
    ord.reserve((size_t)bx * by * tw * th);
    for (uint32_t jj = 0; jj < by; ++jj)
      for (uint32_t i = 0; i < bx; ++i)
        for (uint32_t k = 0; k < tw * th; ++k) {
          const uint32_t j = mode == 1 ? by - 1 - jj : jj;
          const uint32_t x = i * tw + k % tw, y = j * th + k / tw;
          ord.push_back(x < W && y < rows ? y * W + x : kNoPixel);
        }
  }
  return ord;
}
static int ensure_order(ykgpu_context* ctx, uint32_t W, uint32_t rows, uint32_t stride) {
  const uint32_t mode = order_mode();
  if (ctx->d_order && ctx->order_w == W && ctx->order_rows == rows && ctx->order_stride == stride &&
      ctx->order_mode == mode)
    return YK_OK;
  const std::vector<uint32_t> ord = build_order(W, rows, stride, mode);
  if (int rc = quiesce(ctx)) return rc;
  (void)hipFree(ctx->d_order);
  ctx->d_order = nullptr;
  ctx->order_w = ctx->order_rows = ctx->order_slots = 0;
  YK_HIP(hipMalloc(&ctx->d_order, ord.size() * sizeof(uint32_t)));
  YK_HIP(hipMemcpy(ctx->d_order, ord.data(), ord.size() * sizeof(uint32_t), hipMemcpyHostToDevice));
  ctx->order_w = W;
  ctx->order_rows = rows;
  ctx->order_stride = stride;
  ctx->order_mode = mode;
  ctx->order_slots = (uint32_t)ord.size();
  return YK_OK;
}

hipError_t create_render_stream(hipStream_t* s) {
  int least = 0, greatest = 0;
  const char* e = ab_knob("YKGPU_RENDER_PRIO");
  if ((e && std::atoi(e) == 0) || hipDeviceGetStreamPriorityRange(&least, &greatest) != hipSuccess)
    return hipStreamCreateWithFlags(s, hipStreamNonBlocking);
  return hipStreamCreateWithPriority(s, hipStreamNonBlocking, greatest);
}

static uint32_t col_ring() {
  uint32_t r = YK_COL_RING;
  if (const char* e = ab_knob("YKGPU_COL_RING")) r = (uint32_t)std::max(2, std::min(8, std::atoi(e)));
  return r;
}

static uint32_t reduce_blocks(const ykgpu_context* ctx, uint32_t nps) {
  uint32_t cap = (uint32_t)ctx->cus * 4;
  if (const char* e = ab_knob("YKGPU_RED_BLOCKS")) cap = (uint32_t)std::max(0, std::atoi(e));
  const uint32_t full = (nps + 255) / 256;
  return cap ? std::max(1u, std::min(full, cap)) : full;
}

static uint32_t warm_per_cu(bool f32) {
  uint32_t per_cu = f32 ? 2u : (uint32_t)YK_WARM_PER_CU;
  if (const char* e = ab_knob("YKGPU_WARM_PER_CU")) per_cu = (uint32_t)std::max(1, std::atoi(e));
  return per_cu;
}
inline uint32_t warm_blocks_for(uint64_t n, uint64_t cap, uint32_t ilp) {
  uint64_t wb = std::min<uint64_t>((n + 256 * kWarmSlots - 1) / (256 * kWarmSlots), cap);
  if (ilp > 1 && wb > 0) {
    const uint64_t per = 256ull * ilp, it = (n + wb * per - 1) / (wb * per);
    wb = (n + per * it - 1) / (per * it);
  }
  return (uint32_t)wb;
}


struct LaunchPlan {
  bool f32, x128;
  bool group;
  const DevTree* tree;
  const DevTree::Plan* plan;
  int grid, block;
  uint64_t seed_key;
  const uint32_t* order;
  uint32_t nps;
  uint32_t spp;
  std::vector<std::pair<uint32_t, uint32_t>> sched;
  uint64_t shape;
  bool warm_first;
  uint32_t K, nlaunch, kWarmRing, kColRing, mem_shrinks;
  size_t welem;
  uint32_t retry_cap;
  size_t retry_n;
};

static uint64_t warm_wave_slots(const ykgpu_context* ctx, uint64_t nl) {
  const uint64_t wb = warm_blocks_for(nl, (uint64_t)ctx->cus * warm_per_cu(false), kWalkIlp);
  return (nl + wb * 256 - 1) / (wb * 256) * 64;
}

static int plan_launch(ykgpu_context* ctx, const yk_render_params* p, uint32_t s_begin, uint32_t s_end,
                       ykgpu_film* film, LaunchPlan& lp) {
  const bool f32 = lp.f32 = p->precision == YK_PRECISION_FP32;
  const bool x128 = lp.x128 = p->rng == YK_RNG_XOR128;
  const DevTree& tree = *(lp.tree = f32 ? &ctx->t32 : &ctx->t64);
  const DevTree::Plan& plan = *(lp.plan = &tree.plan[x128 ? 1 : 0]);
  const int grid = lp.grid = plan.grid, block = lp.block = block_of(x128);
  int rc = ensure_scratch(ctx, p->max_depth, (size_t)grid * block, !x128);
  if (rc) return rc;
  uint64_t& seed_key = lp.seed_key = 0;
  if (p->seed_mode == YK_SEED_RANDOM_DEVICE) {
    seed_key = p->seed_key;
    if (!seed_key) {
      std::random_device rd;
      while (!seed_key) seed_key = ((uint64_t)rd() << 32) | rd();
    }
  }
  if (!film && (rc = ensure_order(ctx, tile_width(p), p->row_count, order_stride(p)))) return rc;
  const bool group = lp.group = film && film->g_slots != 0;
  lp.order = group ? film->d_gorder : film ? film->d_order : ctx->d_order;
  const uint32_t nps = lp.nps = group ? film->g_slots : film ? film->nps : ctx->order_slots;
  const uint32_t spp = lp.spp = s_end - s_begin;
  const yksched::LaunchSizes sizes = yksched::launch_sizes(nps, spp, (uint64_t)grid * block);
  const uint32_t kideal = sizes.kideal, ksynced = sizes.ksynced, kfloor = sizes.kfloor;
  uint32_t kmax = kideal;
  uint32_t& mem_shrinks = lp.mem_shrinks = 0;
  auto shrink = [&]() {
    kmax = std::max(kfloor, kmax / 2);
    ++mem_shrinks;
  };
  auto grow = [&](auto*& ptr, size_t& cap, size_t need, size_t elem) -> int {
    if (need <= cap && (group || 2 * need >= cap)) return YK_OK;
    if (int q = quiesce(ctx)) return q;
    (void)hipFree(ptr);
    ptr = nullptr;
    cap = 0;
    YK_HIP(hipMalloc((void**)&ptr, need * elem));
    cap = need;
    return YK_OK;
  };
  std::vector<std::pair<uint32_t, uint32_t>>& sched = lp.sched;
  uint64_t& shape = lp.shape = 0;
  bool inflight = false;
  uint32_t &K = lp.K = 0, &nlaunch = lp.nlaunch = 0, &kWarmRing = lp.kWarmRing = 0, &kColRing = lp.kColRing = 0;
  const size_t welem = lp.welem = f32 ? sizeof(StartRecF) : sizeof(StartRec);
  const bool warm_first = lp.warm_first = ab_knob("YKGPU_ABL_WARM_FIRST") != nullptr && !x128;
  for (;;) {
    shape = ((uint64_t)nps << 24) ^ ((uint64_t)kmax << 2) ^ (f32 ? 2u : 0u) ^ (x128 ? 1u : 0u);
    inflight = false;
    if (ctx->prev_enqueued && ctx->prev_ok && !ctx->dirty && ctx->prev_shape == shape && ctx->prev_n > 0 &&
        ctx->lev.size() >= 6ull * ctx->prev_n)
      inflight = hipEventQuery(ctx->lev[6 * (ctx->prev_n - 1) + 5]) == hipErrorNotReady;
    yksched::launch_schedule(sched, spp, s_begin, kmax, ksynced, inflight);
    K = kmax;
    nlaunch = (uint32_t)sched.size();
    kWarmRing = nlaunch > 1 ? kWarmRingDepth : 1;
    if (const char* e = ab_knob("YKGPU_WARM_RING"))
      kWarmRing = (uint32_t)std::min<uint64_t>(kDepRing - 1, (uint64_t)std::max(2, std::atoi(e)));
    if (warm_first) kWarmRing = nlaunch;
    kColRing = nlaunch > 1 ? std::min(col_ring(), kDepRing - 1) : 1;
    const size_t need_warm = x128 ? 0 : (size_t)kWarmRing * nps * K * welem;
    const size_t need_col = (size_t)kColRing * nps * K * kColStride * sizeof(double);
    if (kmax > kfloor && (need_warm > ctx->warm_cap || need_col > ctx->col_cap * sizeof(double))) {
      size_t free_b = 0, total_b = 0;
      if (hipMemGetInfo(&free_b, &total_b) == hipSuccess) {
        const size_t held = ctx->warm_cap + ctx->col_cap * sizeof(double);
        if (need_warm + need_col + kMemReserve > free_b + held) {
          shrink();
          continue;
        }
      }
    }
    rc = x128 ? YK_OK : grow(ctx->d_warm, ctx->warm_cap, need_warm, 1);
    if (!rc) rc = grow(ctx->d_col, ctx->col_cap, (size_t)kColRing * nps * K * kColStride, sizeof(double));
    if (rc == YK_ERR_NOMEM && kmax > kfloor) {
      (void)hipGetLastError();
      shrink();
      continue;
    }
    if (rc) return rc;
    break;
  }
  if (!film && sched.size() > 1 && (rc = grow(ctx->d_acc, ctx->acc_cap, (size_t)nps * 3, sizeof(double)))) return rc;
  const bool lens_defer = !x128 && !f32 && ctx->cam.lens_radius > 0;
  uint32_t& retry_cap = lp.retry_cap = 0;
  if (lens_defer)
    for (const auto& l : sched)
      if (warm_wave_slots(ctx, (uint64_t)nps * l.second) <= kDeferSlots)
        retry_cap = std::max(retry_cap, retry_cap_for(warm_wave_slots(ctx, (uint64_t)nps * l.second)));
  if (mem_shrinks) retry_cap = 0;
#ifdef YK_RETRY_CAP_FORCE
  if (retry_cap) retry_cap = YK_RETRY_CAP_FORCE;
#endif
  size_t& retry_n = lp.retry_n = (size_t)ctx->cus * warm_per_cu(false) * 4u * retry_cap * 3u;
  if (retry_cap && (rc = grow(ctx->d_retry, ctx->retry_cap, retry_n, sizeof(uint4)))) {
    if (rc != YK_ERR_NOMEM) return rc;
    (void)hipGetLastError();
    retry_cap = 0;
    retry_n = 0;
  }
  return YK_OK;
}

struct LaunchArgs {
  KernelArgs ka;
  WarmArgs wa;
  ReduceArgs ra;
  FilmReduceArgs fa;
  FilmMaskedArgs fm;
};

static int fill_args(const ykgpu_context* ctx, const yk_render_params* p, uint8_t* rgb_dev, double* sums_dev,
                     const ykgpu_film* film, const LaunchPlan& lp, LaunchArgs& la) {
  const DevTree& tree = *lp.tree;
  const DevTree::Plan& plan = *lp.plan;
  const int grid = lp.grid, block = lp.block;
  const uint32_t nps = lp.nps, retry_cap = lp.retry_cap;
  const uint32_t* const order = lp.order;
  const uint64_t seed_key = lp.seed_key;
  const bool group = lp.group;
  KernelArgs& ka = la.ka;
  ka.cam = ctx->cam;
  ka.pad_a = 0;
  {
    const yk_camera& c = ctx->cam;
    for (int k = 0; k < 3; ++k) {
      ka.camf.origin[k] = (float)c.origin[k];
      ka.camf.llc[k] = (float)c.lower_left_corner[k];
      ka.camf.horizontal[k] = (float)c.horizontal[k];
      ka.camf.vertical[k] = (float)c.vertical[k];
      ka.camf.lens_u[k] = (float)c.lens_u[k];
      ka.camf.lens_v[k] = (float)c.lens_v[k];
      ka.camf.pad[k] = 0.0f;
    }
    ka.camf.lens_radius = (float)c.lens_radius;
    ka.camf.w = (float)p->image_width;
    ka.camf.h = (float)p->image_height;
  }
  ka.W = p->image_width;
  ka.Wt = tile_width(p);
  ka.col_begin = p->col_count ? p->col_begin : 0;
  ka.col_stride = p->col_count ? p->col_stride : 1;
  ka.col_band = p->col_count ? p->col_band_log2 : 0;
  ka.H = p->image_height;
  ka.spp = p->samples_per_pixel;
  ka.max_depth = p->max_depth;
  ka.seed0 = p->seed0;
  ka.row_begin = p->row_begin;
  ka.row_count = p->row_count;
  ka.row_stride = p->row_stride;
  ka.band_log2 = p->row_band_log2;
  ka.nspheres = ctx->nspheres;
  ka.flags = p->flags;
  ka.id_stride = ctx->id_stride;
  ka.start = nullptr;
  ka.order = order;
  ka.t_min = p->t_min;
  ka.origin_bound = tree.origin_bound;
  ka.inv_w = 1.0 / (double)ka.W;
  ka.inv_h = 1.0 / (double)ka.H;
  ka.w_d = (double)ka.W;
  ka.h_d = (double)ka.H;
  ka.bvh_root = tree.root;
  ka.n_nodes = tree.n_nodes;
  ka.lds_geo_off = tree.geo_off;
  ka.lds_ids_off = tree.ids_off;
  ka.lds_tgeo_off = plan.tgeo_off;
  ka.lds_mat_off = plan.mat_off;
  ka.lds_stack_off = plan.stack_off;
  ka.stack_cap = plan.stack_cap;
  ka.nodes = tree.nodes;
  ka.leaf_geo = (const SphereGeo*)tree.leaf_geo;
  ka.leaf_ids = tree.leaf_ids;
  ka.geo = ctx->d_geo;
  ka.mat = ctx->d_mat;
  ka.geo_f = ctx->d_geo_f;
  ka.seed_mode = p->seed_mode;
  ka.seed_key = seed_key;
  ka.pixel_counter = ctx->d_counter;

  ka.counters = ctx->d_stats;
  ka.trace = ctx->d_trace;
  ka.trace_counts = ctx->d_trace_counts;
  ka.trace_cap = ctx->trace_cap;
  ka.claim_tail = (uint32_t)grid * (uint32_t)(block / 64) * kClaim * kClaimTailFactor;
  if ((ka.flags & YK_FLAG_TRACE_RAYS) && !(ctx->d_trace && (ka.flags & YK_FLAG_COUNT_WORK)))
    return fail(YK_ERR_INVALID, "YK_FLAG_TRACE_RAYS is set by ykgpu_render_trace only");
  WarmArgs& wa = la.wa;
  wa.W = p->image_width;
  wa.Wt = ka.Wt;
  wa.col_begin = ka.col_begin;
  wa.col_stride = ka.col_stride;
  wa.col_band = ka.col_band;
  wa.spp = p->samples_per_pixel;
  wa.seed0 = p->seed0;
  wa.row_begin = p->row_begin;
  wa.row_stride = p->row_stride;
  wa.band_log2 = p->row_band_log2;
  wa.out = ctx->d_warm;
  wa.retry = retry_cap ? ctx->d_retry : nullptr;
  wa.retry_cap = retry_cap;
  wa.retry_pad = 0;
  wa.lens = ctx->cam.lens_radius > 0 ? 1u : 0u;
  wa.H = p->image_height;
  wa.cam = ctx->cam;
  wa.camf = ka.camf;
  wa.w_d = ka.w_d;
  wa.h_d = ka.h_d;
  wa.inv_w = ka.inv_w;
  wa.inv_h = ka.inv_h;
  wa.npix_slots = nps;
  fastdiv(nps, wa.nps_m, wa.nps_sh);
  fastdiv(ka.Wt, wa.w_m, wa.w_sh);
  wa.seed_mode = p->seed_mode;
  wa.seed_key = seed_key;
  wa.order = order;
  ka.npix_slots = nps;
  ka.nps_m = wa.nps_m;
  ka.nps_sh = wa.nps_sh;
  ka.w_m = wa.w_m;
  ka.w_sh = wa.w_sh;
  ka.stack_check = plan.stack_check ? 1u : 0u;
  ReduceArgs& ra = la.ra;
  ra.acc = ctx->d_acc;
  ra.order = order;
  ra.rgb = rgb_dev;
  ra.sums = sums_dev;
  ra.npix_slots = nps;
  ra.spp = p->samples_per_pixel;
  ra.pad0 = ra.pad1 = 0;
  FilmReduceArgs& fa = la.fa = FilmReduceArgs{};
  FilmMaskedArgs& fm = la.fm = FilmMaskedArgs{};
  if (group) {
    fm.plane = film->d_plane;
    fm.count = film->d_count;
    fm.map = film->d_gmap;
    fm.npix_slots = film->nps;
    fm.g_slots = nps;
  } else if (film) {
    fa.plane = film->d_plane;
    fa.order = order;
    fa.npix_slots = nps;
  }
  return YK_OK;
}

static int enqueue_launches(ykgpu_context* ctx, hipStream_t st, uint32_t s_end, const ykgpu_film* film,
                            const LaunchPlan& lp, LaunchArgs& la, uint32_t* launches_out) {
  const bool f32 = lp.f32, x128 = lp.x128, group = lp.group, warm_first = lp.warm_first;
  const DevTree::Plan& plan = *lp.plan;
  const int grid = lp.grid, block = lp.block;
  const uint32_t nps = lp.nps, K = lp.K, nlaunch = lp.nlaunch, kWarmRing = lp.kWarmRing, kColRing = lp.kColRing;
  const size_t welem = lp.welem;
  const std::vector<std::pair<uint32_t, uint32_t>>& sched = lp.sched;
  KernelArgs& ka = la.ka;
  WarmArgs& wa = la.wa;
  ReduceArgs& ra = la.ra;
  FilmReduceArgs& fa = la.fa;
  FilmMaskedArgs& fm = la.fm;
  int rc = YK_OK;
  const uint64_t g0 = ctx->g_next;
  ykgpu_context::RingGeom geom;
  geom.nps = nps;
  geom.K = K;
  geom.welem = welem;
  geom.warm_ring = kWarmRing;
  geom.col_ring = kColRing;
  geom.lanes = (uint64_t)grid * block;
  geom.id_stride = ctx->id_stride;
  geom.warm = ctx->d_warm;
  geom.col = ctx->d_col;
  geom.mt = ctx->d_mt;
  geom.ids = ctx->d_ids;
  const char* ove = std::getenv("YKGPU_OVERLAP");
  const bool same_run = ctx->prev_ok && ctx->prev_geom == geom;
  const bool ov = !x128 && !warm_first && !(ove && std::atoi(ove) == 0) && ctx->prev_ok && ctx->prev_geom == geom &&
                  ctx->run_len >= std::max(kWarmRing, kColRing) && std::max(kWarmRing, kColRing) < kDepRing;
  if (ctx->dirty && (rc = quiesce(ctx))) return rc;
  const bool after_prev = ctx->prev_enqueued && !ctx->dirty && !ov;
  ctx->prev_ok = false;
  ctx->dirty = true;
  if (std::max(nlaunch, kWarmRing) > ctx->counter_cap) {
    if ((rc = quiesce(ctx))) return rc;
    (void)hipFree(ctx->d_counter);
    (void)hipFree(ctx->d_clk);
    ctx->d_counter = nullptr;
    ctx->d_clk = nullptr;
    ctx->counter_cap = 0;
    YK_HIP(hipMalloc(&ctx->d_counter, std::max(nlaunch, kWarmRing) * sizeof(uint32_t)));
    YK_HIP(hipMalloc(&ctx->d_clk, 4ull * std::max(nlaunch, kWarmRing) * sizeof(unsigned long long)));
    ctx->counter_cap = std::max(nlaunch, kWarmRing);
  }
  std::swap(ctx->lev, ctx->lev_prev);
  ctx->lev_prev_used = ctx->lev_used;
  while (ctx->lev.size() < 6ull * nlaunch) {
    hipEvent_t e;
    YK_HIP(hipEventCreate(&e));
    ctx->lev.push_back(e);
  }
  ctx->lev_used = 6 * nlaunch;
  if (after_prev) YK_HIP(hipStreamWaitEvent(st, ctx->lev_prev[6 * (ctx->prev_n - 1) + 5], 0));
  if (x128) YK_HIP(hipMemsetAsync(ctx->d_counter, 0, nlaunch * sizeof(uint32_t), st));
  if (!ov) {
    YK_HIP(hipMemsetAsync(ctx->d_stats, 0, kCounters * sizeof(unsigned long long), st));
    YK_HIP(hipMemsetAsync(ctx->d_stats + 16, 0xff, 2 * sizeof(unsigned long long), st));
  }
  YK_HIP(hipEventRecord(ctx->ev0, st));
  if (ov) {
    YK_HIP(hipMemsetAsync(ctx->d_stats, 0, kCounters * sizeof(unsigned long long), ctx->aux));
    YK_HIP(hipMemsetAsync(ctx->d_stats + 16, 0xff, 2 * sizeof(unsigned long long), ctx->aux));
  } else {
    for (hipStream_t s : {ctx->aux, ctx->red, ctx->alt, ctx->ren}) {
      YK_HIP(hipStreamWaitEvent(s, ctx->ev0, 0));
      if (after_prev) YK_HIP(hipStreamWaitEvent(s, ctx->lev_prev[6 * (ctx->prev_n - 1) + 5], 0));
    }
  }
  while (ctx->gev.size() < 2ull * kDepRing) {
    hipEvent_t e;
    YK_HIP(hipEventCreateWithFlags(&e, hipEventDisableTiming));
    ctx->gev.push_back(e);
  }
  auto gdep = [&](uint64_t g, int which) { return ctx->gev[2 * (g % kDepRing) + which]; };
  auto warm = [&](uint32_t c) -> int {
    hipEvent_t* ev = &ctx->lev[6 * c];
    if (c >= kWarmRing)
      YK_HIP(hipStreamWaitEvent(ctx->aux, ctx->lev[6 * (c - kWarmRing) + 3], 0));
    else if (ov)
      YK_HIP(hipStreamWaitEvent(ctx->aux, gdep(g0 + c - kWarmRing, 0), 0));
    wa.s0 = sched[c].first;
    wa.n = (uint64_t)nps * sched[c].second;
    wa.out = ctx->d_warm + (size_t)((g0 + c) % kWarmRing) * nps * K * welem;
    wa.counter = ctx->d_counter + (g0 + c) % kWarmRing;
    const bool defer = !x128 && !f32 && wa.lens && wa.retry_cap && warm_wave_slots(ctx, wa.n) <= kDeferSlots;
    const uint32_t wblocks = warm_blocks_for(wa.n, (uint64_t)ctx->cus * warm_per_cu(f32), defer ? kWalkIlp : 1u);
    YK_HIP(hipEventRecord(ev[0], ctx->aux));
    if (!x128) {
      if (f32 && wa.lens)
        hipLaunchKernelGGL((yk_mt_warmup<true, true>), dim3(wblocks), dim3(256), 0, ctx->aux, wa);
      else if (f32)
        hipLaunchKernelGGL((yk_mt_warmup<false, true>), dim3(wblocks), dim3(256), 0, ctx->aux, wa);
      else if (defer)
        hipLaunchKernelGGL(yk_mt_warmup_defer, dim3(wblocks), dim3(256), 0, ctx->aux, wa);
      else if (wa.lens)
        hipLaunchKernelGGL((yk_mt_warmup<true, false>), dim3(wblocks), dim3(256), 0, ctx->aux, wa);
      else
        hipLaunchKernelGGL((yk_mt_warmup<false, false>), dim3(wblocks), dim3(256), 0, ctx->aux, wa);
      YK_HIP(hipGetLastError());
    }
    YK_HIP(hipEventRecord(ev[1], ctx->aux));
    return YK_OK;
  };
  for (uint32_t c = 0; c < std::min(kWarmRing, nlaunch); ++c)
    if ((rc = warm(c))) return rc;
  if (warm_first) YK_HIP(hipStreamSynchronize(ctx->aux));
  uint32_t launches = 0;
  for (uint32_t c = 0; c < nlaunch; ++c) {
    hipEvent_t* ev = &ctx->lev[6 * c];
    const uint32_t s0 = sched[c].first, ks = sched[c].second;
    const uint32_t nsl = nps * ks;
    const uint64_t g = g0 + c;
    char* const wring = x128 ? nullptr : ctx->d_warm + (size_t)(g % kWarmRing) * nps * K * welem;
    double* col = ctx->d_col + (size_t)(g % kColRing) * nps * K * kColStride;
    ka.s0 = s0;
    ka.nsl = nsl;
    ka.col = col;
    ka.start = (const void*)wring;
    const hipStream_t rs = (g & 1) ? ctx->alt : ctx->ren;
    const size_t lanes = (size_t)grid * block;
    ka.mt_scratch = ctx->d_mt ? ctx->d_mt + (g & 1) * lanes * ykd::kMtN : nullptr;
    ka.id_scratch = ctx->d_ids + (g & 1) * lanes * ctx->id_stride;
    YK_HIP(hipStreamWaitEvent(rs, ev[1], 0));
    if (c >= kColRing)
      YK_HIP(hipStreamWaitEvent(rs, ctx->lev[6 * (c - kColRing) + 5], 0));
    else if (ov)
      YK_HIP(hipStreamWaitEvent(rs, gdep(g0 + c - kColRing, 1), 0));
    ka.pixel_counter = ctx->d_counter + (x128 ? c : (uint32_t)(g % kWarmRing));
    ka.clk = ctx->d_clk + 4 * c;
#ifdef YK_DRAIN_DIAG
    ka.diag_c = c;
    ka.diag_pad = 0;
#endif
    YK_HIP(hipEventRecord(ev[2], rs));
    const bool count = (ka.flags & YK_FLAG_COUNT_WORK) != 0;
    if (f32)
      hipLaunchKernelGGL(f32_kernel(plan.in_lds, (count ? 1 : 0) | (x128 ? 4 : 0)), dim3(grid), dim3(block),
                         plan.lds_bytes, rs, ka);
    else
      hipLaunchKernelGGL(fp64_kernel(plan.in_lds, (count ? 1 : 0) | (ka.seed_mode == YK_SEED_RANDOM_DEVICE ? 2 : 0) |
                                                      (x128 ? 4 : 0)),
                         dim3(grid), dim3(block), plan.lds_bytes, rs, ka);
    YK_HIP(hipGetLastError());
    YK_HIP(hipEventRecord(ev[3], rs));
    YK_HIP(hipEventRecord(gdep(g, 0), rs));
    ra.col = col;
    ra.nsl = nsl;
    ra.ks = ks;
    ra.first = s0 == 0;
    ra.last = s0 + ks == s_end;
    YK_HIP(hipStreamWaitEvent(ctx->red, ev[3], 0));
    if (ov && !film && ra.last) YK_HIP(hipStreamWaitEvent(ctx->red, ctx->ev0, 0));
    YK_HIP(hipEventRecord(ev[4], ctx->red));
    if (group) {
      fm.col = col;
      fm.ks = ks;
      fm.take = s0 + ks == s_end ? film->d_take : nullptr;
      hipLaunchKernelGGL(yk_film_reduce_masked, dim3(reduce_blocks(ctx, nps)), dim3(256), 0, ctx->red, fm);
    } else if (film) {
      fa.col = col;
      fa.ks = ks;
      hipLaunchKernelGGL(yk_film_reduce, dim3(reduce_blocks(ctx, nps)), dim3(256), 0, ctx->red, fa);
    } else {
      hipLaunchKernelGGL(yk_reduce_samples, dim3(reduce_blocks(ctx, nps)), dim3(256), 0, ctx->red, ra);
    }
    YK_HIP(hipGetLastError());
    YK_HIP(hipEventRecord(ev[5], ctx->red));
    YK_HIP(hipEventRecord(gdep(g, 1), ctx->red));
    if (c + kWarmRing < nlaunch && (rc = warm(c + kWarmRing))) return rc;
    ++launches;
  }
  YK_HIP(hipStreamWaitEvent(st, ctx->lev[6 * (nlaunch - 1) + 5], 0));
  YK_HIP(hipEventRecord(ctx->ev1, st));
  ctx->g_next = g0 + nlaunch;
  ctx->prev_n = nlaunch;
  ctx->run_len = (same_run ? ctx->run_len : 0) + nlaunch;
  ctx->prev_geom = geom;
  ctx->prev_shape = lp.shape;
  ctx->prev_ok = !x128 && !warm_first;
  ctx->prev_enqueued = true;
  ctx->dirty = false;
  *launches_out = launches;
  return YK_OK;
}

static void call_stats(ykgpu_context* ctx, const yk_render_params* p, const double* sums_dev, const ykgpu_film* film,
                       const LaunchPlan& lp, uint32_t launches) {
  const bool x128 = lp.x128;
  const int grid = lp.grid, block = lp.block;
  const uint32_t nps = lp.nps, K = lp.K, nlaunch = lp.nlaunch, kWarmRing = lp.kWarmRing, kColRing = lp.kColRing;
  const size_t welem = lp.welem, retry_n = lp.retry_n;
  const uint32_t retry_cap = lp.retry_cap;
  ctx->stats = yk_render_stats{};
  ctx->stats.samples = (uint64_t)p->row_count * tile_width(p) * lp.spp;
  ctx->stats.launches = launches;
  ctx->stats.grid_blocks = (uint32_t)grid;
  ctx->stats.launch_spp = K;
  ctx->stats.mem_shrinks = lp.mem_shrinks;
  ctx->stats.seed_key = lp.seed_key;
  {
    const uint64_t lanes = (uint64_t)grid * block;
    uint64_t cb = ctx->t64.bytes + ctx->t32.bytes +
                  (uint64_t)ctx->nspheres * (sizeof(SphereGeo) + sizeof(SphereMat) + sizeof(float4));
    cb += (uint64_t)kColRing * nps * K * kColStride * sizeof(double) + (x128 ? 0 : (uint64_t)kWarmRing * nps * K * welem);
    cb += (film ? (uint64_t)nps * 6 * sizeof(double) : nlaunch > 1 ? (uint64_t)nps * 3 * sizeof(double) : 0) +
          (uint64_t)nps * sizeof(uint32_t);
    cb += nlaunch * sizeof(uint32_t) + kCounters * sizeof(unsigned long long);
    if (retry_cap) cb += retry_n * sizeof(uint4);
    if (!x128) cb += 2 * lanes * ykd::kMtN * sizeof(uint32_t);
    cb += 2 * lanes * std::max(1u, p->max_depth > kStackRegs ? p->max_depth : 1u) * sizeof(uint16_t);
    const uint64_t npix = (uint64_t)p->row_count * tile_width(p);
    cb += npix * 3 + (sums_dev ? npix * 3 * sizeof(double) : 0);
    ctx->stats.call_bytes = cb;
  }
  ctx->stats_pending = true;
}

int launch(ykgpu_context* ctx, const yk_render_params* p, uint8_t* rgb_dev, double* sums_dev, hipStream_t st,
           uint32_t s_begin, uint32_t s_end, ykgpu_film* film) {
  LaunchPlan lp;
  LaunchArgs la;
  uint32_t launches = 0;
  int rc = plan_launch(ctx, p, s_begin, s_end, film, lp);
  if (!rc) rc = fill_args(ctx, p, rgb_dev, sums_dev, film, lp, la);
  if (!rc) rc = enqueue_launches(ctx, st, s_end, film, lp, la, &launches);
  if (!rc) call_stats(ctx, p, sums_dev, film, lp, launches);
  return rc;
}

}
```

### uecraytracing_amd/csrc/yk_schedule.hpp

```cpp
#ifndef YK_SCHEDULE_HPP
#define YK_SCHEDULE_HPP

#include <algorithm>
#include <cstddef>
#include <cstdint>
#include <cstdlib>
#include <utility>
#include <vector>

#ifndef YK_LAUNCH_MB
#define YK_LAUNCH_MB 8192
#endif
constexpr uint64_t kLaunchBytes = (uint64_t)YK_LAUNCH_MB << 20;
#ifndef YK_LAUNCH_SPP
#define YK_LAUNCH_SPP 32
#endif
constexpr uint32_t kLaunchSpp = YK_LAUNCH_SPP;
#ifndef YK_LAUNCH_SPP_OV
#define YK_LAUNCH_SPP_OV 64
#endif
constexpr uint32_t kLaunchSppOv = YK_LAUNCH_SPP_OV;
#ifndef YK_LAUNCHES_PER_CALL
#define YK_LAUNCHES_PER_CALL 32
#endif
constexpr uint32_t kLaunchesPerCall = YK_LAUNCHES_PER_CALL;
#ifndef YK_LAUNCH_SLOTS
#define YK_LAUNCH_SLOTS (1u << 26)
#endif
constexpr uint64_t kLaunchSlots = YK_LAUNCH_SLOTS;
#ifndef YK_LAUNCH_SLOTS_OV
#define YK_LAUNCH_SLOTS_OV (1u << 27)
#endif
constexpr uint64_t kLaunchSlotsOv = YK_LAUNCH_SLOTS_OV;
constexpr uint32_t kDepRing = 16;
constexpr uint64_t kMemFloorSlots = 1ull << 24;
constexpr size_t kMemReserve = (size_t)512 << 20;
#ifndef YK_WARM_RING
#define YK_WARM_RING 3
#endif
constexpr uint32_t kWarmRingDepth = YK_WARM_RING;
#ifndef YK_FIRST_LAUNCH
#define YK_FIRST_LAUNCH 4
#endif
constexpr uint32_t kFirstLaunch = YK_FIRST_LAUNCH;
#ifndef YK_SCHED_GROW
#define YK_SCHED_GROW 2
#endif
constexpr uint32_t kSchedGrow = YK_SCHED_GROW;
#ifndef YK_FIRST_LAUNCH_OV
#define YK_FIRST_LAUNCH_OV 0
#endif
#ifndef YK_SCHED_GROW_OV
#define YK_SCHED_GROW_OV 4
#endif
constexpr uint32_t kFirstLaunchOv = YK_FIRST_LAUNCH_OV, kSchedGrowOv = YK_SCHED_GROW_OV;
static_assert(YK_FIRST_LAUNCH >= 1 && YK_LAUNCH_SPP >= 1, "launch sizes must be >= 1 sample per pixel");
#ifndef YK_TILE
#define YK_TILE 8
#endif
constexpr uint32_t kTile = YK_TILE;
#ifndef YK_COL_RING
#define YK_COL_RING 2
#endif
#ifndef YK_WARM_PER_CU
#define YK_WARM_PER_CU 32
#endif
#ifndef YK_WARM_SLOTS
#define YK_WARM_SLOTS 4
#endif
constexpr uint32_t kWarmSlots = YK_WARM_SLOTS;

namespace {
#ifdef YK_AB_KNOBS
inline const char* ab_knob(const char* name) { return std::getenv(name); }
#else
constexpr const char* ab_knob(const char*) { return nullptr; }
#endif
}

namespace yksched {

constexpr uint64_t kColourBytes = 32;

struct LaunchSizes {
  uint32_t kideal, ksynced, kfloor;
};

inline LaunchSizes launch_sizes(uint32_t nps, uint32_t spp, uint64_t lanes) {
  const uint64_t fill_spp = (lanes * 16 + nps - 1) / nps;
  uint64_t launch_slots = kLaunchSlots;
  if (const char* e = ab_knob("YKGPU_LAUNCH_SLOTS")) launch_slots = (uint64_t)std::max(1ll, std::atoll(e));
  auto launches_for = [&](uint64_t lslots) {
    return std::max<uint64_t>(1, ((uint64_t)nps * spp + lslots / 2) / lslots);
  };
  const uint64_t call_launches = launches_for(launch_slots);
  const uint64_t call_launches_ov =
      std::max(std::min<uint64_t>(call_launches, 2), launches_for(std::max(launch_slots, kLaunchSlotsOv)));
  const uint64_t slot_spp = (spp + call_launches - 1) / call_launches;
  const uint64_t slot_spp_ov = (spp + call_launches_ov - 1) / call_launches_ov;
  uint64_t launch_spp = std::max<uint64_t>(kLaunchSpp, spp / kLaunchesPerCall);
  if (const char* e = ab_knob("YKGPU_LAUNCH_SPP")) launch_spp = (uint64_t)std::max(1, std::atoi(e));
  const uint64_t launch_spp_ov = std::max<uint64_t>(std::max<uint64_t>(kLaunchSppOv, launch_spp), spp / kLaunchesPerCall);
  auto ideal_for = [&](uint64_t lspp, uint64_t sspp) {
    return (uint32_t)std::max<uint64_t>(
        1, std::min<uint64_t>({spp, kLaunchBytes / (kColourBytes * nps),
                               std::max<uint64_t>({lspp, fill_spp, sspp}), ((1ull << 31) - 1) / nps}));
  };
  LaunchSizes z;
  z.kideal = ideal_for(launch_spp_ov, slot_spp_ov);
  z.ksynced = ideal_for(launch_spp, slot_spp);
  z.kfloor = (uint32_t)std::min<uint64_t>(z.kideal, std::max<uint64_t>(1, (kMemFloorSlots + nps - 1) / nps));
  return z;
}

inline void launch_schedule(std::vector<std::pair<uint32_t, uint32_t>>& sched, uint32_t spp, uint32_t s_begin,
                            uint32_t kmax, uint32_t ksynced, bool inflight) {
  const uint32_t kcap = inflight ? kmax : std::min(kmax, ksynced);
  uint32_t first_k = inflight ? (kFirstLaunchOv ? kFirstLaunchOv : kmax) : kFirstLaunch;
  uint32_t grow_k = inflight ? kSchedGrowOv : kSchedGrow;
  if (const char* e = ab_knob(inflight ? "YKGPU_FIRST_LAUNCH_OV" : "YKGPU_FIRST_LAUNCH"))
    first_k = (uint32_t)std::max(1, std::atoi(e));
  if (const char* e = ab_knob(inflight ? "YKGPU_SCHED_GROW_OV" : "YKGPU_SCHED_GROW"))
    grow_k = (uint32_t)std::max(2, std::atoi(e));
  sched.clear();
  for (uint32_t s0 = 0, k = std::min(first_k, kcap); s0 < spp;) {
    uint32_t take = std::min(k, spp - s0);
    const uint32_t rest = spp - (s0 + take);
    if (rest > 0 && rest < std::max(1u, take / 4))
      take = spp - s0 <= kcap ? spp - s0 : (spp - s0 + 1) / 2;
    sched.emplace_back(s_begin + s0, take);
    s0 += take;
    k = std::min(grow_k * k, kcap);
  }
}

}

#endif
```

Baseline: 7421 Msamples/s.

## Cull sky-only pixel blocks via camera frustum tests and shade them in a cheap kernel

On the host, each pixel block's view pyramid (widened for the lens aperture) is tested conservatively against every sphere. Blocks whose rays provably hit no sphere are flagged as sky. Those pixels leave the BVH path-tracing pipeline and go to a light kernel that draws the same MT random numbers and computes only the background gradient. Rare lens-rejection overflows fall back to a full Mersenne Twister redo kernel. This saves traversal work on sky pixels, at the cost of host-side geometry tests, extra buffers and stream orchestration, and a risk to bit-exactness if the conservative bounds are ever wrong.

```diff
diff --git a/uecraytracing_amd/csrc/yk_bvh.cpp b/uecraytracing_amd/csrc/yk_bvh.cpp
--- a/uecraytracing_amd/csrc/yk_bvh.cpp
+++ b/uecraytracing_amd/csrc/yk_bvh.cpp
@@ -1,4 +1,6 @@
 #include "yk_bvh.hpp"
+
+#include "yk_sky.hpp"
 
 #include <algorithm>
 #include <cmath>
@@ -339,3 +341,174 @@
 }
 
 }
+
+namespace yksky {
+namespace {
+
+struct V {
+  double x, y, z;
+};
+inline V vsub(V a, V b) { return {a.x - b.x, a.y - b.y, a.z - b.z}; }
+inline V vadd(V a, V b) { return {a.x + b.x, a.y + b.y, a.z + b.z}; }
+inline V vmul(V a, double s) { return {a.x * s, a.y * s, a.z * s}; }
+inline double vdot(V a, V b) { return a.x * b.x + a.y * b.y + a.z * b.z; }
+inline V vcross(V a, V b) { return {a.y * b.z - a.z * b.y, a.z * b.x - a.x * b.z, a.x * b.y - a.y * b.x}; }
+inline double vlen(V a) { return std::sqrt(vdot(a, a)); }
+inline V v3(const double* p) { return {p[0], p[1], p[2]}; }
+
+constexpr double kRel = 1e-9;
+constexpr double kDisc = 0x1p-40;
+
+struct Pyramid {
+  V n[5];
+  double fmin = 0;
+  double cone = 0;
+  V corner[4];
+  bool ok = false;
+};
+
+struct Cam {
+  V o, llc, hor, ver;
+  double L = 0;
+  double scale = 0;
+};
+
+Cam make_cam(const yk_camera& c) {
+  Cam k;
+  k.o = v3(c.origin), k.llc = v3(c.lower_left_corner), k.hor = v3(c.horizontal), k.ver = v3(c.vertical);
+  if (c.lens_radius > 0) {
+    const V lu = v3(c.lens_u), lv = v3(c.lens_v);
+    k.L = c.lens_radius * std::sqrt(vdot(lu, lu) + vdot(lv, lv)) * (1 + kRel);
+  }
+  k.scale = vlen(k.o) + vlen(k.llc) + vlen(k.hor) + vlen(k.ver);
+  return k;
+}
+
+void corners(const Cam& c, double u0, double u1, double v0, double v1, V (&e)[4]) {
+  const double us[4] = {u0, u1, u1, u0}, vs[4] = {v0, v0, v1, v1};
+  for (int k = 0; k < 4; ++k) e[k] = vsub(vadd(vadd(c.llc, vmul(c.hor, us[k])), vmul(c.ver, vs[k])), c.o);
+}
+
+Pyramid make_pyramid(const Cam& c, double u0, double u1, double v0, double v1) {
+  Pyramid p;
+  V in[4];
+  corners(c, u0 - kRel / 2, u1 + kRel / 2, v0 - kRel / 2, v1 + kRel / 2, in);
+  const double need = c.L * (1 + kRel);
+  V w = vadd(vadd(in[0], in[1]), vadd(in[2], in[3]));
+  const double wl = vlen(w);
+  if (!(wl > 0) || !std::isfinite(wl)) return p;
+  w = vmul(w, 1.0 / wl);
+  double fmin = INFINITY;
+  for (int k = 0; k < 4; ++k) fmin = std::min(fmin, vdot(w, in[k]));
+  if (!(fmin * (1 - kRel) > need) || !std::isfinite(fmin)) return p;
+  double cmin = 1.0;
+  for (int k = 0; k < 4; ++k) cmin = std::min(cmin, vdot(w, in[k]) / vlen(in[k]));
+  p.cone = std::acos(std::max(-1.0, std::min(1.0, cmin))) + std::asin(need / (fmin * (1 - kRel))) + kRel;
+  if (!std::isfinite(p.cone)) return p;
+  const double hl = vlen(c.hor), vl = vlen(c.ver);
+  for (double g = 1.0 + 0x1p-20; g <= 32.0; g *= (need > 0 ? 1.0625 : 64.0)) {
+    const double du = kRel + g * c.L / hl, dv = kRel + g * c.L / vl;
+    if (!std::isfinite(du) || !std::isfinite(dv)) return p;
+    V e[4];
+    corners(c, u0 - du, u1 + du, v0 - dv, v1 + dv, e);
+    bool good = true;
+    for (int k = 0; k < 4 && good; ++k) {
+      V n = vcross(e[k], e[(k + 1) & 3]);
+      const double len = vlen(n);
+      if (!(len > 0) || !std::isfinite(len)) return p;
+      n = vmul(n, 1.0 / len);
+      if (vdot(n, w) < 0) n = vmul(n, -1.0);
+      for (int j = 0; j < 4 && good; ++j) good = vdot(n, in[j]) >= need && vdot(n, in[j]) > 0;
+      p.n[k] = n;
+    }
+    if (!good) continue;
+    p.n[4] = w;
+    p.fmin = fmin * (1 - kRel);
+    for (int k = 0; k < 4; ++k) p.corner[k] = in[k];
+    p.ok = true;
+    return p;
+  }
+  return p;
+}
+
+bool excluded(const Cam& c, const Pyramid& p, V C, double r) {
+  if (!p.ok) return false;
+  const V oc = vsub(C, c.o);
+  const double D = vlen(oc), ar = std::fabs(r);
+  const double reach = D + ar + c.L;
+  const double tmax = reach / (p.fmin - c.L);
+  const double rho = (ar + c.L) * (1 + kRel) + kRel * (reach + (1 + tmax) * c.scale) + kDisc * reach * reach / ar;
+  if (!(rho >= 0) || !std::isfinite(rho)) return false;
+  for (int k = 0; k < 5; ++k)
+    if (vdot(p.n[k], oc) < -rho) return true;
+  if (D - c.L > rho - c.L && D > c.L) {
+    const double theta = std::acos(std::max(-1.0, std::min(1.0, vdot(p.n[4], oc) / D)));
+    const double need = p.cone + std::asin(c.L / D) + std::asin((rho - c.L) / (D - c.L)) + kRel;
+    if (theta > need) return true;
+  }
+  return false;
+}
+
+bool covered(const Cam& c, const Pyramid& p, V C, double r) {
+  if (!p.ok) return false;
+  const V oc = vsub(C, c.o);
+  const double tan2 = vdot(oc, oc) - r * r;
+  if (!(tan2 > 0)) return false;
+  for (int k = 0; k < 4; ++k) {
+    const double a = vdot(p.corner[k], oc);
+    if (!(a > 0) || !(a * a > tan2 * vdot(p.corner[k], p.corner[k]) * (1 + 1e-6))) return false;
+  }
+  return true;
+}
+
+inline uint64_t banded(uint32_t begin, uint32_t stride, uint32_t L, uint32_t t) {
+  return (uint64_t)begin + ((((uint64_t)(t >> L)) * stride) << L) + (t & ((1u << L) - 1u));
+}
+
+}
+
+std::vector<uint8_t> sky_blocks(const yk_camera& cam, const double* centers, const double* radii, uint32_t n,
+                                const Tile& t, uint32_t tw, uint32_t th) {
+  const uint32_t bx = (t.col_count + tw - 1) / tw, by = (t.row_count + th - 1) / th;
+  std::vector<uint8_t> flag((size_t)bx * by, 0);
+  if (!bx || !by || !t.W || !t.H) return flag;
+  const Cam c = make_cam(cam);
+  const double W = (double)t.W, H = (double)t.H;
+  auto pyramid = [&](uint32_t j0, uint32_t j1, uint32_t r0, uint32_t r1) {
+    const double x0 = (double)banded(t.col_begin, t.col_stride, t.col_band_log2, j0);
+    const double x1 = (double)banded(t.col_begin, t.col_stride, t.col_band_log2, j1 - 1);
+    const double y0 = (double)banded(t.row_begin, t.row_stride, t.row_band_log2, r0);
+    const double y1 = (double)banded(t.row_begin, t.row_stride, t.row_band_log2, r1 - 1);
+    return make_pyramid(c, x0 / W, (x1 + 1) / W, (H - 1 - y1) / H, (H - y0) / H);
+  };
+  constexpr uint32_t kSuper = 8;
+  std::vector<uint32_t> left;
+  for (uint32_t sj = 0; sj < by; sj += kSuper)
+    for (uint32_t si = 0; si < bx; si += kSuper) {
+      const uint32_t ei = std::min(bx, si + kSuper), ej = std::min(by, sj + kSuper);
+      const Pyramid sp = pyramid(si * tw, std::min(t.col_count, ei * tw), sj * th, std::min(t.row_count, ej * th));
+      left.clear();
+      bool hidden = false;
+      for (uint32_t s = 0; s < n && !hidden; ++s) {
+        if (excluded(c, sp, v3(centers + 3 * (size_t)s), radii[s])) continue;
+        left.push_back(s);
+        hidden = covered(c, sp, v3(centers + 3 * (size_t)s), radii[s]);
+      }
+      if (hidden) continue;
+      for (uint32_t j = sj; j < ej; ++j)
+        for (uint32_t i = si; i < ei; ++i) {
+          bool sky = sp.ok;
+          if (!left.empty()) {
+            const Pyramid bp =
+                pyramid(i * tw, std::min(t.col_count, (i + 1) * tw), j * th, std::min(t.row_count, (j + 1) * th));
+            sky = bp.ok;
+            for (size_t k = 0; sky && k < left.size(); ++k)
+              sky = excluded(c, bp, v3(centers + 3 * (size_t)left[k]), radii[left[k]]);
+          }
+          flag[(size_t)j * bx + i] = sky ? 1 : 0;
+        }
+    }
+  return flag;
+}
+
+}
diff --git a/uecraytracing_amd/csrc/yk_context.hip b/uecraytracing_amd/csrc/yk_context.hip
--- a/uecraytracing_amd/csrc/yk_context.hip
+++ b/uecraytracing_amd/csrc/yk_context.hip
@@ -44,6 +44,7 @@
   b += ctx->retry_cap * sizeof(uint4);
   b += (uint64_t)ctx->order_slots * sizeof(uint32_t) + (uint64_t)ctx->counter_cap * sizeof(uint32_t);
   b += kCounters * sizeof(unsigned long long);
+  b += sky_bytes(ctx);
   if (ctx->d_mt) b += 2ull * ctx->scratch_lanes * ykd::kMtN * sizeof(uint32_t);
   if (ctx->d_ids) b += 2ull * ctx->id_lanes * ctx->id_stride * sizeof(uint16_t);
   b += ctx->rgb_cap + ctx->sums_cap * sizeof(double);
@@ -283,6 +284,12 @@
   (void)hipFree(ctx->d_order);
   (void)hipFree(ctx->d_col);
   (void)hipFree(ctx->d_acc);
+  (void)hipFree(ctx->d_sky_path);
+  (void)hipFree(ctx->d_sky_list);
+  (void)hipFree(ctx->d_sky_acc);
+  (void)hipFree(ctx->d_sky_mt);
+  (void)hipFree(ctx->d_sky_off);
+  if (ctx->sky_ev) (void)hipEventDestroy(ctx->sky_ev);
   ctx->t64.release();
   ctx->t32.release();
   (void)hipFree(ctx->d_mt);
@@ -408,6 +415,8 @@
   YK_HIP(hipStreamSynchronize(ctx->stream));
   ctx->nspheres = count;
   ctx->cam = *camera;
+  ctx->sky_centers = centers;
+  ctx->sky_radii = radii;
   double ext = 0;
   for (uint32_t i = 0; i < count; ++i) {
     const yk_sphere& s = spheres[i];
diff --git a/uecraytracing_amd/csrc/yk_device.hpp b/uecraytracing_amd/csrc/yk_device.hpp
--- a/uecraytracing_amd/csrc/yk_device.hpp
+++ b/uecraytracing_amd/csrc/yk_device.hpp
@@ -195,6 +195,12 @@
   }
   return x;
 }
+__device__ __forceinline__ void mt_twist(uint32_t* st) {
+  uint32_t k = 0;
+  for (; k < kMtN - kMtM; ++k) st[k] = st[k + kMtM] ^ mt_mix(st[k], st[k + 1]);
+  for (; k < kMtN - 1; ++k) st[k] = st[k + kMtM - kMtN] ^ mt_mix(st[k], st[k + 1]);
+  st[kMtN - 1] = st[kMtM - 1] ^ mt_mix(st[kMtN - 1], st[0]);
+}
 __device__ __noinline__ uint32_t mt_slow(uint32_t* st, uint32_t x227, uint32_t j) {
   const uint32_t idx = j % kMtN;
   if (j == kLazyDraws) {
@@ -205,13 +211,31 @@
       st[i] = x;
     }
   }
-  if (j == kLazyDraws || idx == 0) {
-    uint32_t k = 0;
-    for (; k < kMtN - kMtM; ++k) st[k] = st[k + kMtM] ^ mt_mix(st[k], st[k + 1]);
-    for (; k < kMtN - 1; ++k) st[k] = st[k + kMtM - kMtN] ^ mt_mix(st[k], st[k + 1]);
-    st[kMtN - 1] = st[kMtM - 1] ^ mt_mix(st[kMtN - 1], st[0]);
-  }
+  if (j == kLazyDraws || idx == 0) mt_twist(st);
   return st[idx];
+}
+
+struct MtFull {
+  uint32_t* st;
+  uint32_t idx, n;
+};
+__device__ inline void mt_full_seed(MtFull& g, uint32_t seed) {
+  uint32_t x = seed;
+  g.st[0] = x;
+  for (uint32_t i = 1; i < kMtN; ++i) {
+    x = mt_seed_step(x, i);
+    g.st[i] = x;
+  }
+  g.idx = kMtN;
+  g.n = 0;
+}
+__device__ inline uint32_t mt_full_next(MtFull& g) {
+  if (g.idx >= kMtN) {
+    mt_twist(g.st);
+    g.idx = 0;
+  }
+  ++g.n;
+  return mt_temper(g.st[g.idx++]);
 }
 
 __device__ __forceinline__ uint32_t mt_next_lazy(MtLane& g) {
@@ -282,6 +306,8 @@
 __device__ __forceinline__ uint32_t rng_next(MtLane& g) { return kLazy ? mt_next_lazy(g) : mt_next(g); }
 template <bool kLazy = false>
 __device__ __forceinline__ uint32_t rng_next(X128Lane& g) { return x128_next(g); }
+template <bool kLazy = false>
+__device__ __forceinline__ uint32_t rng_next(MtFull& g) { return mt_full_next(g); }
 
 template <bool kLazy = false, class G>
 __device__ __forceinline__ double canonical(G& g) {
diff --git a/uecraytracing_amd/csrc/yk_host_internal.hpp b/uecraytracing_amd/csrc/yk_host_internal.hpp
--- a/uecraytracing_amd/csrc/yk_host_internal.hpp
+++ b/uecraytracing_amd/csrc/yk_host_internal.hpp
@@ -71,6 +71,16 @@
   uint32_t* d_order = nullptr;
   uint32_t order_w = 0, order_rows = 0, order_slots = 0, order_stride = 0, order_mode = 0;
   size_t warm_cap = 0;
+  std::vector<double> sky_centers, sky_radii;
+  std::vector<uint64_t> sky_key;
+  uint32_t* d_sky_path = nullptr;
+  uint32_t* d_sky_list = nullptr;
+  double* d_sky_acc = nullptr;
+  uint32_t* d_sky_mt = nullptr;
+  uint32_t* d_sky_off = nullptr;
+  size_t sky_cap = 0;
+  uint32_t sky_path_slots = 0, sky_slots = 0, sky_full_slots = 0;
+  hipEvent_t sky_ev = nullptr;
   hipStream_t stream = nullptr;
   hipStream_t aux = nullptr;
   hipStream_t red = nullptr;
@@ -208,6 +218,13 @@
 hipError_t create_render_stream(hipStream_t* s);
 int launch(ykgpu_context* ctx, const yk_render_params* p, uint8_t* rgb_dev, double* sums_dev, hipStream_t st,
            uint32_t s_begin, uint32_t s_end, ykgpu_film* film);
+constexpr uint32_t kSkyEngines = 64;
+inline uint64_t sky_bytes(const ykgpu_context* ctx) {
+  if (!ctx->sky_cap) return 0;
+  const uint64_t full = ctx->sky_cap;
+  return (full + 256 + full + full / 64 + 1 + full + (uint64_t)kSkyEngines * ykd::kMtN) * sizeof(uint32_t) +
+         full * 3 * sizeof(double);
+}
 uint64_t device_bytes(const ykgpu_context* ctx);
 int finish_stats(ykgpu_context* ctx);
 int film_ready(const ykgpu_film* film);
diff --git a/uecraytracing_amd/csrc/yk_pipeline.hip b/uecraytracing_amd/csrc/yk_pipeline.hip
--- a/uecraytracing_amd/csrc/yk_pipeline.hip
+++ b/uecraytracing_amd/csrc/yk_pipeline.hip
@@ -11,6 +11,7 @@
 #include "yk_film_internal.hpp"
 #include "yk_host_internal.hpp"
 #include "yk_schedule.hpp"
+#include "yk_sky.hpp"
 
 namespace {
 
@@ -251,6 +252,18 @@
   uint32_t npix_slots, nsl, ks, spp;
   uint32_t first, last, pad0, pad1;
 };
+__device__ __forceinline__ void pixel_store(double* sums, uint8_t* rgb, uint32_t q, const double (&a)[3],
+                                            uint32_t spp_u) {
+  const size_t o3 = (size_t)q * 3;
+  const double spp = (double)spp_u;
+#pragma unroll
+  for (int c = 0; c < 3; ++c) {
+    if (sums) sums[o3 + c] = a[c];
+    double v = ykd::nsqrt(a[c] / spp);
+    v = (v < 0.0) ? 0.0 : (0.999 < v) ? 0.999 : v;
+    rgb[o3 + c] = (uint8_t)(uint32_t)(v * 256);
+  }
+}
 __device__ __forceinline__ void reduce_slot(const ReduceArgs& ra, uint32_t p) {
   const uint32_t q = ra.order[p];
   if (q == kNoPixel) return;
@@ -267,19 +280,132 @@
     for (int c = 0; c < 3; ++c) ra.acc[(size_t)c * ra.npix_slots + p] = a[c];
     return;
   }
-  const size_t o3 = (size_t)q * 3;
-  const double spp = (double)ra.spp;
-#pragma unroll
-  for (int c = 0; c < 3; ++c) {
-    if (ra.sums) ra.sums[o3 + c] = a[c];
-    double v = ykd::nsqrt(a[c] / spp);
-    v = (v < 0.0) ? 0.0 : (0.999 < v) ? 0.999 : v;
-    ra.rgb[o3 + c] = (uint8_t)(uint32_t)(v * 256);
-  }
+  pixel_store(ra.sums, ra.rgb, q, a, ra.spp);
 }
 __global__ __launch_bounds__(256) void yk_reduce_samples(ReduceArgs ra) {
   for (uint32_t p = blockIdx.x * blockDim.x + threadIdx.x; p < ra.npix_slots; p += gridDim.x * blockDim.x)
     reduce_slot(ra, p);
+}
+
+struct SkyArgs {
+  uint32_t W, H, spp, seed0, row_begin, row_stride, band_log2;
+  uint32_t Wt, col_begin, col_stride, col_band;
+  uint32_t w_m, w_sh;
+  uint32_t lens, s0, ks, first, last;
+  uint32_t n;
+  yk_camera cam;
+  double w_d, h_d, inv_w, inv_h;
+  const uint32_t* list;
+  double* acc;
+  uint8_t* rgb;
+  double* sums;
+  uint32_t* engines;
+  unsigned long long* counters;
+};
+__device__ __forceinline__ void sky_add(const SkyArgs& sa, uint32_t xx, uint32_t y, double uc, double vc, double px,
+                                        double py, double (&a)[3]) {
+  v3 o, d;
+  camera_ray(sa.cam, sa.w_d, sa.inv_w, sa.h_d, sa.inv_h, sa.H, xx, y, uc, vc, sa.lens != 0, px, py, o, d);
+  const double len = ykd::nsqrt(ykd::len2(d));
+  const v3 un = ykd::divs_fast(d, len);
+  const double t = (un.y + 1.0) / 2;
+  a[0] = a[0] + ((1.0 - t) * 1.0 + t * 0.5);
+  a[1] = a[1] + ((1.0 - t) * 1.0 + t * 0.7);
+  a[2] = a[2] + ((1.0 - t) * 1.0 + t * 1.0);
+}
+#ifndef YK_SKY_LAZY_WORDS
+#define YK_SKY_LAZY_WORDS ykd::kLazyDraws
+#endif
+__global__ __launch_bounds__(256) __attribute__((amdgpu_num_vgpr(YK_DEFER_VGPRS / 2))) void yk_sky_samples(SkyArgs sa) {
+  const uint32_t p = blockIdx.x * 256u + threadIdx.x;
+  if (p >= sa.n) return;
+  const uint32_t q = sa.list[p];
+  if (q == kNoPixel) return;
+  const uint32_t tr = fdiv(q, sa.w_m, sa.w_sh);
+  const uint32_t xx = tile_col_x(sa.col_begin, sa.col_stride, sa.col_band, q - tr * sa.Wt);
+  const uint32_t y = tile_row_y(sa.row_begin, sa.row_stride, sa.band_log2, tr);
+  const uint32_t seed_s0 = ykd::sample_seed(0u, 0ull, sa.seed0, y, xx, sa.W, sa.spp, sa.s0);
+  double a[3];
+#pragma unroll
+  for (int c = 0; c < 3; ++c) a[c] = sa.first ? 0.0 : sa.acc[(size_t)c * sa.n + p];
+  for (uint32_t k = 0; k < sa.ks; k += kWalkIlp) {
+    uint32_t x[kWalkIlp];
+#pragma unroll
+    for (uint32_t j = 0; j < kWalkIlp; ++j) x[j] = seed_s0 + k + j;
+    ykd::mt_walk397xn<kWalkIlp>(x);
+#pragma unroll
+    for (uint32_t j = 0; j < kWalkIlp; ++j) {
+      if (k + j >= sa.ks) break;
+      ykd::MtLane g;
+      g.state = nullptr;
+      ykd::mt_start_from(g, seed_s0 + k + j, x[j]);
+      const double uc = ykd::canonical<true>(g);
+      const double vc = ykd::canonical<true>(g);
+      double px = 0.0, py = 0.0;
+      if (sa.lens) {
+        for (;;) {
+          if (g.j + 4 > YK_SKY_LAZY_WORDS) {
+            sa.engines[1 + atomicAdd(sa.engines, 1u)] = p;
+            return;
+          }
+          px = ykd::uniform<true>(g, -1, 1);
+          py = ykd::uniform<true>(g, -1, 1);
+          if (px * px + py * py < 1.0) break;
+        }
+      }
+      sky_add(sa, xx, y, uc, vc, px, py, a);
+    }
+  }
+  if (!sa.last) {
+#pragma unroll
+    for (int c = 0; c < 3; ++c) sa.acc[(size_t)c * sa.n + p] = a[c];
+    return;
+  }
+  pixel_store(sa.sums, sa.rgb, q, a, sa.spp);
+}
+__global__ __launch_bounds__(64) __attribute__((amdgpu_num_vgpr(YK_DEFER_VGPRS / 2))) void yk_sky_redo(SkyArgs sa) {
+  const uint32_t count = sa.engines[0];
+  uint32_t fallbacks = 0;
+  ykd::MtFull g;
+  g.st = sa.engines + 1 + sa.n + (size_t)threadIdx.x * ykd::kMtN;
+  for (uint32_t e = threadIdx.x; e < count; e += 64u) {
+    const uint32_t p = sa.engines[1 + e], q = sa.list[p];
+    const uint32_t tr = fdiv(q, sa.w_m, sa.w_sh);
+    const uint32_t xx = tile_col_x(sa.col_begin, sa.col_stride, sa.col_band, q - tr * sa.Wt);
+    const uint32_t y = tile_row_y(sa.row_begin, sa.row_stride, sa.band_log2, tr);
+    double a[3];
+#pragma unroll
+    for (int c = 0; c < 3; ++c) a[c] = sa.first ? 0.0 : sa.acc[(size_t)c * sa.n + p];
+    for (uint32_t k = 0; k < sa.ks; ++k) {
+      ykd::mt_full_seed(g, ykd::sample_seed(0u, 0ull, sa.seed0, y, xx, sa.W, sa.spp, sa.s0 + k));
+      const double uc = ykd::canonical(g);
+      const double vc = ykd::canonical(g);
+      double px, py;
+      do {
+        px = ykd::uniform(g, -1, 1);
+        py = ykd::uniform(g, -1, 1);
+      } while (!(px * px + py * py < 1.0));
+      if (g.n > ykd::kLazyDraws) ++fallbacks;
+      sky_add(sa, xx, y, uc, vc, px, py, a);
+    }
+    if (sa.last) {
+      pixel_store(sa.sums, sa.rgb, q, a, sa.spp);
+    } else {
+#pragma unroll
+      for (int c = 0; c < 3; ++c) sa.acc[(size_t)c * sa.n + p] = a[c];
+    }
+  }
+  if (fallbacks) atomicAdd(&sa.counters[3], (unsigned long long)fallbacks);
+  __syncthreads();
+  if (threadIdx.x == 0) sa.engines[0] = 0u;
+}
+
+__global__ __launch_bounds__(256) void yk_sky_split(const uint32_t* order, const uint32_t* off, uint32_t* path,
+                                                    uint32_t* list, uint32_t n, uint32_t per) {
+  const uint32_t i = blockIdx.x * 256u + threadIdx.x;
+  if (i >= n) return;
+  const uint32_t b = i / per, o = off[b];
+  ((o & 0x80000000u) ? list : path)[(size_t)(o & 0x7fffffffu) * per + (i - b * per)] = order[i];
 }
 
 struct FilmReduceArgs {
@@ -448,8 +574,8 @@
     ord.resize((size_t)W * rows);
     for (size_t i = 0; i < ord.size(); ++i) ord[i] = (uint32_t)i;
   } else {
-    const uint32_t th = stride <= 1 ? kTile : (stride <= 4 ? std::max(1u, kTile / 2) : std::max(1u, kTile / 4));
-    const uint32_t tw = kTile * kTile / th;
+    uint32_t tw, th;
+    order_block(stride, tw, th);
     const uint32_t bx = (W + tw - 1) / tw, by = (rows + th - 1) / th;
     ord.reserve((size_t)bx * by * tw * th);
     for (uint32_t jj = 0; jj < by; ++jj)
@@ -482,6 +608,73 @@
   return YK_OK;
 }
 
+static bool sky_eligible(const yk_render_params* p, const ykgpu_film* film, const DevTree::Plan& plan) {
+  if (const char* e = ab_knob("YKGPU_SKY"))
+    if (std::atoi(e) == 0) return false;
+  return kTile != 0 && !film && p->precision == YK_PRECISION_FP64 && p->rng == YK_RNG_MT19937 &&
+         p->seed_mode == YK_SEED_COUNTER && p->flags == 0 && p->max_depth > 0 && plan.in_lds;
+}
+static int ensure_sky(ykgpu_context* ctx, const yk_render_params* p) {
+  const uint32_t Wt = tile_width(p), rows = p->row_count, stride = order_stride(p), mode = order_mode();
+  const uint32_t col_begin = p->col_count ? p->col_begin : 0, col_stride = p->col_count ? p->col_stride : 1;
+  const uint32_t col_band = p->col_count ? p->col_band_log2 : 0;
+  const std::vector<uint64_t> key = {ctx->scene_gen, p->image_width, p->image_height, p->row_begin, rows,
+                                     p->row_stride,  p->row_band_log2, col_begin,     Wt,           col_stride,
+                                     col_band,       stride,           mode};
+  if (ctx->sky_key == key) return YK_OK;
+  if (int rc = ensure_order(ctx, Wt, rows, stride)) return rc;
+  uint32_t tw, th;
+  order_block(stride, tw, th);
+  const yksky::Tile tile{p->image_width, p->image_height, p->row_begin, rows,       p->row_stride,
+                         p->row_band_log2, col_begin,      Wt,           col_stride, col_band};
+  const std::vector<uint8_t> flag = yksky::sky_blocks(ctx->cam, ctx->sky_centers.data(), ctx->sky_radii.data(),
+                                                      ctx->nspheres, tile, tw, th);
+  const uint32_t bx = (Wt + tw - 1) / tw, by = (rows + th - 1) / th, per = tw * th;
+  std::vector<uint32_t> off((size_t)bx * by);
+  uint32_t npath = 0, nlist = 0;
+  for (uint32_t jj = 0; jj < by; ++jj)
+    for (uint32_t i = 0; i < bx; ++i) {
+      const uint32_t j = mode == 1 ? by - 1 - jj : jj;
+      off[(size_t)jj * bx + i] = flag[(size_t)j * bx + i] ? (0x80000000u | nlist++) : npath++;
+    }
+  ctx->sky_key.clear();
+  ctx->sky_path_slots = ctx->sky_slots = ctx->sky_full_slots = 0;
+  if (nlist) {
+    const size_t full = ctx->order_slots;
+    if (int rc = quiesce(ctx)) return rc;
+    if (full > ctx->sky_cap) {
+      for (void* q : {(void*)ctx->d_sky_path, (void*)ctx->d_sky_list, (void*)ctx->d_sky_acc, (void*)ctx->d_sky_mt,
+                      (void*)ctx->d_sky_off})
+        (void)hipFree(q);
+      ctx->d_sky_path = ctx->d_sky_list = ctx->d_sky_mt = ctx->d_sky_off = nullptr;
+      ctx->d_sky_acc = nullptr;
+      ctx->sky_cap = 0;
+      YK_HIP(hipMalloc(&ctx->d_sky_path, (full + 256) * sizeof(uint32_t)));
+      YK_HIP(hipMalloc(&ctx->d_sky_list, full * sizeof(uint32_t)));
+      YK_HIP(hipMalloc(&ctx->d_sky_acc, full * 3 * sizeof(double)));
+      YK_HIP(hipMalloc(&ctx->d_sky_mt, (1 + full + (size_t)kSkyEngines * ykd::kMtN) * sizeof(uint32_t)));
+      YK_HIP(hipMalloc(&ctx->d_sky_off, off.size() * sizeof(uint32_t)));
+      ctx->sky_cap = full;
+    }
+    if (!ctx->sky_ev) YK_HIP(hipEventCreateWithFlags(&ctx->sky_ev, hipEventDisableTiming));
+    const size_t path_slots = ((size_t)npath * per + 255) / 256 * 256;
+    YK_HIP(hipMemcpy(ctx->d_sky_off, off.data(), off.size() * sizeof(uint32_t), hipMemcpyHostToDevice));
+    hipLaunchKernelGGL(yk_sky_split, dim3((uint32_t)((full + 255) / 256)), dim3(256), 0, ctx->stream, ctx->d_order,
+                       ctx->d_sky_off, ctx->d_sky_path, ctx->d_sky_list, (uint32_t)full, per);
+    YK_HIP(hipGetLastError());
+    if (path_slots > (size_t)npath * per)
+      YK_HIP(hipMemsetAsync(ctx->d_sky_path + (size_t)npath * per, 0xff, (path_slots - (size_t)npath * per) * 4,
+                            ctx->stream));
+    YK_HIP(hipMemsetAsync(ctx->d_sky_mt, 0, sizeof(uint32_t), ctx->stream));
+    YK_HIP(hipStreamSynchronize(ctx->stream));
+    ctx->sky_path_slots = (uint32_t)path_slots;
+    ctx->sky_slots = nlist * per;
+    ctx->sky_full_slots = (uint32_t)full;
+  }
+  ctx->sky_key = key;
+  return YK_OK;
+}
+
 hipError_t create_render_stream(hipStream_t* s) {
   int least = 0, greatest = 0;
   const char* e = ab_knob("YKGPU_RENDER_PRIO");
@@ -508,7 +701,12 @@
   if (const char* e = ab_knob("YKGPU_WARM_PER_CU")) per_cu = (uint32_t)std::max(1, std::atoi(e));
   return per_cu;
 }
-inline uint32_t warm_blocks_for(uint64_t n, uint64_t cap, uint32_t ilp) {
+inline uint32_t warm_blocks_for(uint64_t n, uint64_t cap, uint32_t ilp, uint64_t align = 0) {
+  if (align && align / 256 <= cap && n % align == 0) {
+    const uint64_t m = align / 256, ks = n / align;
+    for (uint64_t j = std::min(cap / m, ks / ilp); j >= 1; --j)
+      if (ks % (j * ilp) == 0 && ks / j >= kWarmSlots) return (uint32_t)(j * m);
+  }
   uint64_t wb = std::min<uint64_t>((n + 256 * kWarmSlots - 1) / (256 * kWarmSlots), cap);
   if (ilp > 1 && wb > 0) {
     const uint64_t per = 256ull * ilp, it = (n + wb * per - 1) / (wb * per);
@@ -521,6 +719,8 @@
 struct LaunchPlan {
   bool f32, x128;
   bool group;
+  bool culled;
+  uint64_t warm_align;
   const DevTree* tree;
   const DevTree::Plan* plan;
   int grid, block;
@@ -537,8 +737,8 @@
   size_t retry_n;
 };
 
-static uint64_t warm_wave_slots(const ykgpu_context* ctx, uint64_t nl) {
-  const uint64_t wb = warm_blocks_for(nl, (uint64_t)ctx->cus * warm_per_cu(false), kWalkIlp);
+static uint64_t warm_wave_slots(const ykgpu_context* ctx, uint64_t nl, uint64_t align) {
+  const uint64_t wb = warm_blocks_for(nl, (uint64_t)ctx->cus * warm_per_cu(false), kWalkIlp, align);
   return (nl + wb * 256 - 1) / (wb * 256) * 64;
 }
 
@@ -559,12 +759,22 @@
       while (!seed_key) seed_key = ((uint64_t)rd() << 32) | rd();
     }
   }
-  if (!film && (rc = ensure_order(ctx, tile_width(p), p->row_count, order_stride(p)))) return rc;
+  bool& culled = lp.culled = false;
+  if (sky_eligible(p, film, plan)) {
+    if ((rc = ensure_sky(ctx, p))) return rc;
+    culled = ctx->sky_slots != 0;
+  }
+  if (!film && !culled && (rc = ensure_order(ctx, tile_width(p), p->row_count, order_stride(p)))) return rc;
   const bool group = lp.group = film && film->g_slots != 0;
-  lp.order = group ? film->d_gorder : film ? film->d_order : ctx->d_order;
-  const uint32_t nps = lp.nps = group ? film->g_slots : film ? film->nps : ctx->order_slots;
+  lp.order = group ? film->d_gorder : film ? film->d_order : culled ? ctx->d_sky_path : ctx->d_order;
+  const uint32_t nps = lp.nps = group    ? film->g_slots
+                                : film   ? film->nps
+                                : culled ? ctx->sky_path_slots
+                                         : ctx->order_slots;
+  lp.warm_align = culled ? nps : 0;
   const uint32_t spp = lp.spp = s_end - s_begin;
-  const yksched::LaunchSizes sizes = yksched::launch_sizes(nps, spp, (uint64_t)grid * block);
+  const yksched::LaunchSizes sizes =
+      yksched::launch_sizes(culled ? ctx->sky_full_slots : nps, spp, (uint64_t)grid * block);
   const uint32_t kideal = sizes.kideal, ksynced = sizes.ksynced, kfloor = sizes.kfloor;
   uint32_t kmax = kideal;
   uint32_t& mem_shrinks = lp.mem_shrinks = 0;
@@ -597,13 +807,15 @@
     yksched::launch_schedule(sched, spp, s_begin, kmax, ksynced, inflight);
     K = kmax;
     nlaunch = (uint32_t)sched.size();
+    if (nps == 0) break;
     kWarmRing = nlaunch > 1 ? kWarmRingDepth : 1;
     if (const char* e = ab_knob("YKGPU_WARM_RING"))
       kWarmRing = (uint32_t)std::min<uint64_t>(kDepRing - 1, (uint64_t)std::max(2, std::atoi(e)));
     if (warm_first) kWarmRing = nlaunch;
     kColRing = nlaunch > 1 ? std::min(col_ring(), kDepRing - 1) : 1;
-    const size_t need_warm = x128 ? 0 : (size_t)kWarmRing * nps * K * welem;
-    const size_t need_col = (size_t)kColRing * nps * K * kColStride * sizeof(double);
+    const size_t nps_ring = culled ? ctx->sky_full_slots : nps;
+    const size_t need_warm = x128 ? 0 : (size_t)kWarmRing * nps_ring * K * welem;
+    const size_t need_col = (size_t)kColRing * nps_ring * K * kColStride * sizeof(double);
     if (kmax > kfloor && (need_warm > ctx->warm_cap || need_col > ctx->col_cap * sizeof(double))) {
       size_t free_b = 0, total_b = 0;
       if (hipMemGetInfo(&free_b, &total_b) == hipSuccess) {
@@ -615,7 +827,7 @@
       }
     }
     rc = x128 ? YK_OK : grow(ctx->d_warm, ctx->warm_cap, need_warm, 1);
-    if (!rc) rc = grow(ctx->d_col, ctx->col_cap, (size_t)kColRing * nps * K * kColStride, sizeof(double));
+    if (!rc) rc = grow(ctx->d_col, ctx->col_cap, (size_t)kColRing * nps_ring * K * kColStride, sizeof(double));
     if (rc == YK_ERR_NOMEM && kmax > kfloor) {
       (void)hipGetLastError();
       shrink();
@@ -624,13 +836,15 @@
     if (rc) return rc;
     break;
   }
-  if (!film && sched.size() > 1 && (rc = grow(ctx->d_acc, ctx->acc_cap, (size_t)nps * 3, sizeof(double)))) return rc;
-  const bool lens_defer = !x128 && !f32 && ctx->cam.lens_radius > 0;
+  if (!film && nps && sched.size() > 1 && (rc = grow(ctx->d_acc, ctx->acc_cap, (size_t)(culled ? ctx->sky_full_slots : nps) * 3, sizeof(double))))
+    return rc;
+  const bool lens_defer = !x128 && !f32 && nps && ctx->cam.lens_radius > 0;
   uint32_t& retry_cap = lp.retry_cap = 0;
   if (lens_defer)
     for (const auto& l : sched)
-      if (warm_wave_slots(ctx, (uint64_t)nps * l.second) <= kDeferSlots)
-        retry_cap = std::max(retry_cap, retry_cap_for(warm_wave_slots(ctx, (uint64_t)nps * l.second)));
+      if (warm_wave_slots(ctx, (uint64_t)nps * l.second, lp.warm_align) <= kDeferSlots)
+        retry_cap =
+            std::max(retry_cap, retry_cap_for(warm_wave_slots(ctx, (uint64_t)nps * l.second, lp.warm_align)));
   if (mem_shrinks) retry_cap = 0;
 #ifdef YK_RETRY_CAP_FORCE
   if (retry_cap) retry_cap = YK_RETRY_CAP_FORCE;
@@ -651,6 +865,7 @@
   ReduceArgs ra;
   FilmReduceArgs fa;
   FilmMaskedArgs fm;
+  SkyArgs sa;
 };
 
 static int fill_args(const ykgpu_context* ctx, const yk_render_params* p, uint8_t* rgb_dev, double* sums_dev,
@@ -753,7 +968,7 @@
   wa.inv_w = ka.inv_w;
   wa.inv_h = ka.inv_h;
   wa.npix_slots = nps;
-  fastdiv(nps, wa.nps_m, wa.nps_sh);
+  fastdiv(std::max(nps, 1u), wa.nps_m, wa.nps_sh);
   fastdiv(ka.Wt, wa.w_m, wa.w_sh);
   wa.seed_mode = p->seed_mode;
   wa.seed_key = seed_key;
@@ -785,6 +1000,62 @@
     fa.order = order;
     fa.npix_slots = nps;
   }
+  SkyArgs& sa = la.sa = SkyArgs{};
+  if (lp.culled) {
+    sa.W = ka.W, sa.H = ka.H, sa.spp = ka.spp, sa.seed0 = ka.seed0;
+    sa.row_begin = ka.row_begin, sa.row_stride = ka.row_stride, sa.band_log2 = ka.band_log2;
+    sa.Wt = ka.Wt, sa.col_begin = ka.col_begin, sa.col_stride = ka.col_stride, sa.col_band = ka.col_band;
+    sa.w_m = ka.w_m, sa.w_sh = ka.w_sh;
+    sa.lens = wa.lens;
+    sa.n = ctx->sky_slots;
+    sa.cam = ctx->cam;
+    sa.w_d = ka.w_d, sa.h_d = ka.h_d, sa.inv_w = ka.inv_w, sa.inv_h = ka.inv_h;
+    sa.list = ctx->d_sky_list;
+    sa.acc = ctx->d_sky_acc;
+    sa.rgb = rgb_dev;
+    sa.sums = sums_dev;
+    sa.engines = ctx->d_sky_mt;
+    sa.counters = ctx->d_stats;
+  }
+  return YK_OK;
+}
+
+static int enqueue_sky(ykgpu_context* ctx, hipStream_t s, SkyArgs& sa, uint32_t s0, uint32_t ks, uint32_t s_end,
+                       bool wait_caller) {
+  sa.s0 = s0;
+  sa.ks = ks;
+  sa.first = s0 == 0;
+  sa.last = s0 + ks == s_end;
+  if (sa.last && wait_caller) YK_HIP(hipStreamWaitEvent(s, ctx->ev0, 0));
+  hipLaunchKernelGGL(yk_sky_samples, dim3((sa.n + 255) / 256), dim3(256), 0, s, sa);
+  YK_HIP(hipGetLastError());
+  if (sa.lens) {
+    hipLaunchKernelGGL(yk_sky_redo, dim3(1), dim3(kSkyEngines), 0, s, sa);
+    YK_HIP(hipGetLastError());
+  }
+  return YK_OK;
+}
+
+static int enqueue_sky_only(ykgpu_context* ctx, hipStream_t st, uint32_t s_begin, uint32_t s_end, LaunchArgs& la) {
+  int rc = YK_OK;
+  if (ctx->dirty && (rc = quiesce(ctx))) return rc;
+  if (ctx->prev_enqueued && ctx->prev_n > 0)
+    YK_HIP(hipStreamWaitEvent(st, ctx->lev[6 * (ctx->prev_n - 1) + 5], 0));
+  ctx->prev_ok = false;
+  ctx->dirty = true;
+  YK_HIP(hipMemsetAsync(ctx->d_stats, 0, kCounters * sizeof(unsigned long long), st));
+  YK_HIP(hipMemsetAsync(ctx->d_stats + 16, 0xff, 2 * sizeof(unsigned long long), st));
+  YK_HIP(hipEventRecord(ctx->ev0, st));
+  YK_HIP(hipStreamWaitEvent(ctx->red, ctx->ev0, 0));
+  if ((rc = enqueue_sky(ctx, ctx->red, la.sa, s_begin, s_end - s_begin, s_end, false))) return rc;
+  YK_HIP(hipEventRecord(ctx->sky_ev, ctx->red));
+  YK_HIP(hipStreamWaitEvent(st, ctx->sky_ev, 0));
+  YK_HIP(hipEventRecord(ctx->ev1, st));
+  ctx->lev_used = 0;
+  ctx->prev_n = 0;
+  ctx->run_len = 0;
+  ctx->prev_enqueued = false;
+  ctx->dirty = false;
   return YK_OK;
 }
 
@@ -874,8 +1145,10 @@
     wa.n = (uint64_t)nps * sched[c].second;
     wa.out = ctx->d_warm + (size_t)((g0 + c) % kWarmRing) * nps * K * welem;
     wa.counter = ctx->d_counter + (g0 + c) % kWarmRing;
-    const bool defer = !x128 && !f32 && wa.lens && wa.retry_cap && warm_wave_slots(ctx, wa.n) <= kDeferSlots;
-    const uint32_t wblocks = warm_blocks_for(wa.n, (uint64_t)ctx->cus * warm_per_cu(f32), defer ? kWalkIlp : 1u);
+    const bool defer =
+        !x128 && !f32 && wa.lens && wa.retry_cap && warm_wave_slots(ctx, wa.n, lp.warm_align) <= kDeferSlots;
+    const uint32_t wblocks =
+        warm_blocks_for(wa.n, (uint64_t)ctx->cus * warm_per_cu(f32), defer ? kWalkIlp : 1u, lp.warm_align);
     YK_HIP(hipEventRecord(ev[0], ctx->aux));
     if (!x128) {
       if (f32 && wa.lens)
@@ -940,6 +1213,7 @@
     ra.ks = ks;
     ra.first = s0 == 0;
     ra.last = s0 + ks == s_end;
+    if (lp.culled && (rc = enqueue_sky(ctx, ctx->red, la.sa, s0, ks, s_end, ov))) return rc;
     YK_HIP(hipStreamWaitEvent(ctx->red, ev[3], 0));
     if (ov && !film && ra.last) YK_HIP(hipStreamWaitEvent(ctx->red, ctx->ev0, 0));
     YK_HIP(hipEventRecord(ev[4], ctx->red));
@@ -998,6 +1272,7 @@
           (uint64_t)nps * sizeof(uint32_t);
     cb += nlaunch * sizeof(uint32_t) + kCounters * sizeof(unsigned long long);
     if (retry_cap) cb += retry_n * sizeof(uint4);
+    if (lp.culled) cb += sky_bytes(ctx) - (uint64_t)nps * sizeof(uint32_t);
     if (!x128) cb += 2 * lanes * ykd::kMtN * sizeof(uint32_t);
     cb += 2 * lanes * std::max(1u, p->max_depth > kStackRegs ? p->max_depth : 1u) * sizeof(uint16_t);
     const uint64_t npix = (uint64_t)p->row_count * tile_width(p);
@@ -1014,7 +1289,10 @@
   uint32_t launches = 0;
   int rc = plan_launch(ctx, p, s_begin, s_end, film, lp);
   if (!rc) rc = fill_args(ctx, p, rgb_dev, sums_dev, film, lp, la);
-  if (!rc) rc = enqueue_launches(ctx, st, s_end, film, lp, la, &launches);
+  if (!rc && lp.culled && lp.nps == 0)
+    rc = enqueue_sky_only(ctx, st, s_begin, s_end, la);
+  else if (!rc)
+    rc = enqueue_launches(ctx, st, s_end, film, lp, la, &launches);
   if (!rc) call_stats(ctx, p, sums_dev, film, lp, launches);
   return rc;
 }
diff --git a/uecraytracing_amd/csrc/yk_schedule.hpp b/uecraytracing_amd/csrc/yk_schedule.hpp
--- a/uecraytracing_amd/csrc/yk_schedule.hpp
+++ b/uecraytracing_amd/csrc/yk_schedule.hpp
@@ -59,6 +59,10 @@
 #define YK_TILE 8
 #endif
 constexpr uint32_t kTile = YK_TILE;
+inline void order_block(uint32_t stride, uint32_t& tw, uint32_t& th) {
+  th = stride <= 1 ? kTile : (stride <= 4 ? std::max(1u, kTile / 2) : std::max(1u, kTile / 4));
+  tw = kTile * kTile / std::max(1u, th);
+}
 #ifndef YK_COL_RING
 #define YK_COL_RING 2
 #endif
diff --git a/uecraytracing_amd/csrc/yk_sky.hpp b/uecraytracing_amd/csrc/yk_sky.hpp
--- /dev/null
+++ b/uecraytracing_amd/csrc/yk_sky.hpp
@@ -0,0 +1,19 @@
+#pragma once
+
+#include <cstdint>
+#include <vector>
+
+#include "../../include/ykgpu.h"
+
+namespace yksky {
+
+struct Tile {
+  uint32_t W, H;
+  uint32_t row_begin, row_count, row_stride, row_band_log2;
+  uint32_t col_begin, col_count, col_stride, col_band_log2;
+};
+
+std::vector<uint8_t> sky_blocks(const yk_camera& cam, const double* centers, const double* radii, uint32_t n,
+                                const Tile& t, uint32_t tw, uint32_t th);
+
+}
```

Result: faster. 7560 Msamples/s (median of 6 runs) (+1.9%).
